# Woody5962/Ranked-List-Truncation

Hardware: AMD Instinct MI355X
Metric: ranked-lists/sec (fwd+bwd) at len=300; F1@k vs CPU ref (higher is better)
Workload: dtype f32 (operands, accumulation, storage); products by exact 3xbf16 split, 6 MFMA products, per-product error < 2^-23; 1 GPU; AttnCut + DivLoss(js,f1,augmented) [BASELINE configs[1]], batch 4096 lists/GPU x len 300, full train step incl. Adam and cut metrics; global_batch=4096, seq_len=300, parallelism=dp1

## Files before the change

include/rlt_hip.h:

```cpp
#ifndef RLT_HIP_H
#define RLT_HIP_H

#include <stddef.h>
#include <stdint.h>

#ifdef __cplusplus
extern "C" {
#endif

#define RLT_E_ARG      (-1)
#define RLT_E_SHAPE    (-2)
#define RLT_E_WORKSPACE (-3)
#define RLT_E_ALIGN    (-4)

#define RLT_ABI_VERSION 5
int rlt_abi_version(void);
#define RLT_PRECISION_DEFAULT (-1)
#define RLT_PRECISION_FP32   0
#define RLT_PRECISION_BF16X3 1
#define RLT_PRECISION_BF16X6 2
int rlt_set_precision(int mode);
int rlt_get_precision(void);
const char* rlt_error_string(int code);

#define RLT_METRIC_F1  0
#define RLT_METRIC_DCG 1
#define RLT_LOSS_EXPECT 0
#define RLT_LOSS_CE     1
#define RLT_LOSS_KL     2
#define RLT_LOSS_JS     3
int rlt_reward_loss(const float* p, const float* labels, const float* dcg_coef, int B, int S,
                    int metric, int kind, float tau,
                    float* loss_per_list, float* loss_out, float* dp, void* stream);
int rlt_reward_loss_ex(const float* p, const float* labels, const float* dcg_coef, int B, int S,
                       int metric, float penalty, int kind, float tau,
                       float* loss_per_list, float* loss_out, float* dp, void* stream);
int rlt_reward_matrix(const float* labels, const float* dcg_coef, int B, int S, int metric, float tau,
                      float* r_out, float* q_out, void* stream);
int rlt_reward_matrix_ex(const float* labels, const float* dcg_coef, int B, int S, int metric, float penalty, float tau,
                         float* r_out, float* q_out, void* stream);
size_t rlt_dcg_table_bytes(void);
int rlt_dcg_table_init(void* table, size_t table_bytes, void* stream);
size_t rlt_loss_metrics_workspace(int B);
int rlt_loss_metrics(const float* p, const float* labels, const float* dcg_coef, int B, int S,
                     int metric, float penalty, int kind, float tau, double metric_penalty,
                     float* loss_per_list, float* loss_out, float* dp,
                     int32_t* k_out, double* f1_out, double* dcg_out, double* sums,
                     const void* dcg_table, void* ws, size_t ws_bytes, void* stream);

size_t rlt_mt_terms_workspace(int B, int S);
int rlt_mt_terms(const float* rerank, const float* cls, const float* labels, int B, int S, float margin,
                 float* terms, void* ws, size_t ws_bytes, void* stream);
int rlt_mt_terms_bwd(const float* cls, const float* labels, const float* terms, int B, int S,
                     float w_rerank, float w_class, const float* gscale,
                     float* d_rerank, float* d_class, void* stream);
int rlt_weighted_sum(const float* const* x, const float* w, int n, float* out, void* stream);

int rlt_cut_metrics(const float* p, const float* labels, const int32_t* k_in, int B, int S,
                    int32_t* k_out, double* f1_out, double* dcg_out, double* sums, void* stream);
int rlt_cut_metrics_ex(const float* p, const float* labels, const int32_t* k_in, int B, int S, double penalty,
                       int32_t* k_out, double* f1_out, double* dcg_out, double* sums, void* stream);

int rlt_task_metrics(const float* labels, const float* pred, int B, int S,
                     double* dcg_out, double* auc_out, double* sums, void* stream);

size_t rlt_truncation_curves_workspace(int B, int S);
int rlt_truncation_curves(const float* labels, int B, int S, double penalty, const void* dcg_table, int accumulate,
                          double* curves, double* best_f1, int32_t* best_f1_k, double* best_dcg, int32_t* best_dcg_k,
                          double* sums, void* ws, size_t ws_bytes, void* stream);

#define RLT_CUT_ARGMAX 0
#define RLT_CUT_PAIR   1
size_t rlt_cut_report_workspace(int B, int S);
int rlt_cut_report(const float* p, int rule, const float* labels, const float* dcg_coef, int B, int S, int metric, float penalty,
                   double metric_penalty, double tau, double sharpen, const void* dcg_table, int accumulate,
                   int32_t* k, float* p_k, float* margin, double* f1, double* dcg, double* best_f1, int32_t* best_f1_k,
                   double* best_dcg, int32_t* best_dcg_k, int32_t* better, double* hist, double* pred_curve, double* reward_curve,
                   double* sums, void* ws, size_t ws_bytes, void* stream);

#define RLT_GEMM_RELU       1
#define RLT_GEMM_ACCUMULATE 2
size_t rlt_gemm_workspace(int ta, int tb, int M, int N, int K);
int rlt_gemm(int ta, int tb, int M, int N, int K,
             const float* A, int lda, const float* B, int ldb, float* C, int ldc,
             const float* bias, const float* bias2, int flags,
             void* ws, size_t ws_bytes, int precision, void* stream);
int rlt_gemm_ex(int ta, int tb, int M, int N, int K,
                const float* A, int lda, const float* B, int ldb, float* C, int ldc,
                const float* bias, const float* bias2, int flags,
                const float* relu_mask, int ldmask, float mask_scale, float* colsum_a,
                float drop_p, uint32_t seed,
                void* ws, size_t ws_bytes, int precision, void* stream);

#define RLT_GEMM_NONE   0
#define RLT_GEMM_F32    1
#define RLT_GEMM_3      2
#define RLT_GEMM_3B     3
#define RLT_GEMM_6      4
#define RLT_GEMM_6B     5
#define RLT_GEMM_6C     6
#define RLT_GEMM_6E     7
#define RLT_GEMM_6S     8
typedef struct rlt_gemm_dispatch {
    int family, ta, tb, fast, persistent, ns, kchunk, slab_xcd, epilogue, narrow;
} rlt_gemm_dispatch;
int rlt_gemm_last_dispatch(rlt_gemm_dispatch* out);

size_t rlt_gemm_bits_words(int M, int N);
int rlt_gemm_bits(int ta, int tb, int M, int N, int K,
                  const float* A, int lda, const float* B, int ldb, float* C, int ldc,
                  const float* bias, int flags, float drop_p, uint32_t seed,
                  uint32_t* relu_bits_out, const uint32_t* mask_bits_in, float mask_scale,
                  int precision, void* stream);
size_t rlt_colsum_workspace(int T, int N);
int rlt_colsum(const float* X, int ldx, int T, int N, float* out, int accumulate,
               void* ws, size_t ws_bytes, void* stream);
int rlt_segment_colsum(const float* X, int ldx, int G, int R, int N, float* out, int ldo,
                       int accumulate, void* stream);

size_t rlt_narrow_dw_workspace(int T, int M);
int rlt_narrow_dw(const float* A, int lda, const float* X, int ldx, int I, int T, int M,
                  float* dW, float* db, void* ws, size_t ws_bytes, void* stream);
int rlt_relu_bwd(float* dX, const float* Y, size_t n, void* stream);
int rlt_scale(float* x, const float* scale, size_t n, void* stream);

int rlt_add_layernorm_fwd(const float* x, const float* r, const float* gamma, const float* beta,
                          int T, int E, float eps, float drop_p, uint32_t seed,
                          float* y, float* stats, void* stream);
size_t rlt_add_layernorm_bwd_workspace(int T, int E);
int rlt_add_layernorm_bwd(const float* x, const float* r, const float* gamma, const float* stats,
                          const float* dy, int T, int E, float drop_p, uint32_t seed,
                          float* dz, float* dr, float* dgamma, float* dbeta,
                          int accumulate, void* ws, size_t ws_bytes, void* stream);
int rlt_dropout_mask(uint32_t seed, size_t rows, int cols, float p, float* out, void* stream);

size_t rlt_list_attention_fwd_workspace(int S, int B, int H, int HD, float drop_p, int precision);
int rlt_list_attention_images_retained(int S, int B, int H, int HD, int precision);
int rlt_list_attention_fwd(const float* qkv, int S, int B, int H, int HD, float drop_p, uint32_t seed,
                           float* out, float* lse, void* images, size_t images_bytes, int precision, void* stream);
size_t rlt_list_attention_bwd_workspace(int S, int B, int H, int HD, float drop_p, int precision);
int rlt_list_attention_bwd(const float* qkv, const float* out, const float* dout, const float* lse,
                           int S, int B, int H, int HD, float drop_p, uint32_t seed, const void* images, float* dqkv,
                           void* ws, size_t ws_bytes, int precision, void* stream);
int rlt_list_attention_bwd_prepare(const float* out, const float* dout, const float* lse, int S, int B, int H, int HD, float drop_p,
                                   const void* images, void* ws, size_t ws_bytes, int precision, void* stream);
int rlt_list_attention_bwd_dkv(const float* qkv, const float* dout, const float* lse, const void* images, void* ws, size_t ws_bytes,
                               int S, int B, int H, int HD, float drop_p, uint32_t seed, float* dqkv, int precision, void* stream);
int rlt_list_attention_bwd_dq(const float* qkv, const float* dout, const float* lse, const void* images, void* ws, size_t ws_bytes,
                              int S, int B, int H, int HD, float drop_p, uint32_t seed, float* dqkv, int precision, void* stream);
#define RLT_ATTN_NONE           0
#define RLT_ATTN_F32            1
#define RLT_ATTN_F32_SB         2
#define RLT_ATTN_F32_OCC1       3
#define RLT_ATTN_F32_HD16       4
#define RLT_ATTN_X3             5
#define RLT_ATTN_X6             6
#define RLT_ATTN_X6_IMG         7
#define RLT_ATTN_X6_PP          8
#define RLT_ATTN_X6_PP_IMG      9
#define RLT_ATTN_X6_DKV1        10
#define RLT_ATTN_X6_DQ1         11
#define RLT_ATTN_X6N_2W         12
#define RLT_ATTN_X6N_2W_SEEDED  13
#define RLT_ATTN_X6N_PIPE       14
#define RLT_ATTN_X6H_PIPE       15
#define RLT_ATTN_PREP_Q      1
#define RLT_ATTN_PREP_K      2
#define RLT_ATTN_PREP_V      4
#define RLT_ATTN_PREP_DO     8
#define RLT_ATTN_PREP_SEEDS  16
#define RLT_ATTN_PREP_DELTA  32
#define RLT_ATTN_IMAGES_NONE    0
#define RLT_ATTN_IMAGES_X3_QKV  1
#define RLT_ATTN_IMAGES_X6_QKV  2
#define RLT_ATTN_IMAGES_X6N_KV  3
#define RLT_ATTN_IMAGES_X6H_KV  4
#define RLT_ATTN_WS_DELTA       0
#define RLT_ATTN_WS_X3_DO       1
#define RLT_ATTN_WS_X6_DO       2
#define RLT_ATTN_WS_X6N_BLOCKS  3
typedef struct rlt_attention_plan {
    int fwd, fwd_fixup, dkv, dq;
    int fwd_prepare, bwd_prepare, dkv_prepare, dq_prepare;
    int images_kind, images_retained, ws_kind;
    size_t images_bytes, flags_offset, flags_bytes;
    size_t delta_bytes, ws_extra_bytes, ws_bytes, ws_prepare_bytes, ws_part_bytes;
} rlt_attention_plan;
int rlt_list_attention_plan(int S, int B, int H, int HD, float drop_p, int have_images, int precision, rlt_attention_plan* out);
int rlt_attention_dropout_mask(uint32_t seed, int S, int B, int H, float p, float* out, void* stream);
int rlt_attention_dropout_mask_range(uint32_t seed, int pair0, int npair, int B, float p, float* out, void* stream);

int rlt_bilstm_rec_fwd(float* gates, const float* w_hh_fwd, const float* w_hh_rev, int S, int B,
                       float* h_out, float* c_out, int precision, void* stream);

int rlt_bilstm_rec_fwd_x(const float* x, int I, const float* w_ih_fwd, const float* b_ih_fwd, const float* b_hh_fwd,
                         const float* w_ih_rev, const float* b_ih_rev, const float* b_hh_rev,
                         const float* w_hh_fwd, const float* w_hh_rev, int S, int B,
                         float* gates, float* h_out, float* c_out, int precision, void* stream);
int rlt_bilstm_rec_bwd(float* gates, const float* c, const float* w_hh_fwd, const float* w_hh_rev,
                       const float* d_hout, int S, int B, int precision, void* stream);
#define RLT_LSTM_F32          1
#define RLT_LSTM_X3           2
#define RLT_LSTM_X6           3
#define RLT_LSTM_X6W_SINGLE   4
#define RLT_LSTM_X6W_HALVES   5
struct rlt_bilstm_rec_plan { int fwd, bwd, fwd_lists, bwd_lists; };
int rlt_bilstm_rec_plan(int B, int xin, int precision, struct rlt_bilstm_rec_plan* out);

#define RLT_OP_ENCODER_STASH   1
#define RLT_OP_ENCODER_FWD_WS  2
#define RLT_OP_ENCODER_BWD_WS  3
#define RLT_OP_BILSTM_STASH    4
#define RLT_OP_BILSTM_WS       5
size_t rlt_workspace_bytes(int op, int S, int B, int E, int H, int FF, int train_dropout, int precision);

typedef struct rlt_encoder_weights {
    const float *in_proj_weight, *in_proj_bias, *out_proj_weight, *out_proj_bias, *norm1_weight, *norm1_bias,
                *linear1_weight, *linear1_bias, *linear2_weight, *linear2_bias, *norm2_weight, *norm2_bias;
} rlt_encoder_weights;
typedef struct rlt_encoder_grads {
    float *in_proj_weight, *in_proj_bias, *out_proj_weight, *out_proj_bias, *norm1_weight, *norm1_bias,
          *linear1_weight, *linear1_bias, *linear2_weight, *linear2_bias, *norm2_weight, *norm2_bias;
} rlt_encoder_grads;
int rlt_encoder_layer_fwd(const float* x, const rlt_encoder_weights* w, int S, int B, int E, int H, int FF, float eps,
                          float drop_p, const uint32_t* seeds, float* y, void* stash, size_t stash_bytes,
                          void* ws, size_t ws_bytes, int precision, void* stream);
int rlt_encoder_layer_bwd(const float* x, const rlt_encoder_weights* w, int S, int B, int E, int H, int FF, float eps,
                          float drop_p, const uint32_t* seeds, const float* dy, const void* stash, size_t stash_bytes,
                          float* dx, const rlt_encoder_grads* g, void* ws, size_t ws_bytes, int precision, void* stream);

typedef struct rlt_lstm_layer_weights { const float *w_ih[2], *w_hh[2], *b_ih[2], *b_hh[2]; } rlt_lstm_layer_weights;
typedef struct rlt_lstm_layer_grads { float *w_ih[2], *w_hh[2], *b_ih[2], *b_hh[2]; } rlt_lstm_layer_grads;
int rlt_bilstm_fwd(const float* x, int I, const rlt_lstm_layer_weights* w, int S, int B, float* h_out,
                   void* stash, size_t stash_bytes, void* ws, size_t ws_bytes, int precision, void* stream);
int rlt_bilstm_bwd(const float* x, int I, const rlt_lstm_layer_weights* w, const float* h_out, const float* dh_out, int S, int B,
                   void* stash, size_t stash_bytes, float* dx, const rlt_lstm_layer_grads* g,
                   void* ws, size_t ws_bytes, int precision, void* stream);

size_t rlt_bilstm_generic_bytes(int stash, int S, int B, int I, int hidden);
int rlt_bilstm_generic_fwd(const float* x, int I, int hidden, const rlt_lstm_layer_weights* w, int S, int B, float* h_out,
                           void* stash, size_t stash_bytes, void* ws, size_t ws_bytes, int precision, void* stream);
int rlt_bilstm_generic_bwd(const float* x, int I, int hidden, const rlt_lstm_layer_weights* w, const float* h_out,
                           const float* dh_out, int S, int B, void* stash, size_t stash_bytes, float* dx,
                           const rlt_lstm_layer_grads* g, void* ws, size_t ws_bytes, int precision, void* stream);

#define RLT_SPARSE_CHUNK 256
typedef struct rlt_sparse_batch {
    const float* dense; const int32_t* ids; const int32_t* perm;
    const int64_t* indptr; const int32_t* indices; const float* values;
    const int64_t* col_ptr; const int32_t* col_rows; const float* col_vals;
    const int32_t *chunk_col, *chunk_ptr, *multi_cols;
    int Dn, n_docs, V, n_chunks, n_multi;
} rlt_sparse_batch;
size_t rlt_sparse_inproj_workspace(int S, int B, int Dn, int n_docs, int V, int n_chunks);
int rlt_sparse_inproj_fwd(const rlt_sparse_batch* sb, int S, int B, const float* wt_fwd, const float* wt_rev,
                          const float* b_ih_fwd, const float* b_hh_fwd, const float* b_ih_rev, const float* b_hh_rev,
                          float* gates, void* stream);
int rlt_sparse_inproj_bwd(const rlt_sparse_batch* sb, int S, int B, const float* dgates, float* dwt_fwd, float* dwt_rev,
                          float* db_ih_fwd, float* db_hh_fwd, float* db_ih_rev, float* db_hh_rev,
// ... 115 lines not shown
```

ranked-list-truncation_amd/csrc/gemm.hip:

```cpp
#include "common.h"
#include "gemm6s.h"
#include "split6.h"
#include <stdlib.h>
#include <string.h>
#include <type_traits>

namespace {

constexpr int BM = 128, BN = 128, LDT = 132;

struct GemmArgs {
    const float* A; const float* B; float* C;
    const float* bias; const float* bias2;
    int M, N, K, lda, ldb, ldc;
    int vecA, vecB;
    int flags;
    int kchunk;
    float* slab;
    int tiles_m, tiles_n;
    const float* mask; int ldmask;
    float* colsum;
    float* cs_slab;
    float drop_p; uint32_t drop_thr, seed;
    float mask_scale;
    int slab_xcd;
    uint32_t* bits_out;
    const uint32_t* bits_in;
    int ldbits;
};

inline void note_dispatch(int family, bool ta, bool tb, bool fast, bool persistent, const GemmArgs& g, int ns) {
    rlt_gemm_dispatch_rec = rlt_gemm_dispatch{family, ta ? 1 : 0, tb ? 1 : 0, fast ? 1 : 0, persistent ? 1 : 0,
                                              ns, g.kchunk, g.slab_xcd, 0, 0};
}

__device__ __forceinline__ void decode_block(const GemmArgs& g, int& bid, int& z) {
    const int nwg = g.tiles_m * g.tiles_n;
    const int id = blockIdx.x;
    if (g.slab_xcd) {
        const int xcd = id & 7, j = id >> 3, grp = j / nwg;
        z = grp * 8 + xcd;
        bid = j - grp * nwg;
    } else {
        const int q = nwg >> 3, r = nwg & 7, xcd = id & 7, j = id >> 3;
        bid = (xcd < r ? xcd * (q + 1) : r * (q + 1) + (xcd - r) * q) + j;
        z = blockIdx.z;
    }
}

__device__ __forceinline__ float gemm_epilogue(const GemmArgs& g, float v, float bv, int row, int col, const float* dst) {
    v += bv;
    if (g.flags & RLT_GEMM_ACCUMULATE) v += *dst;
    if (g.flags & RLT_GEMM_RELU) v = fmaxf(v, 0.f);
    if (g.mask) v = (g.mask[(size_t)row * g.ldmask + col] > 0.f) ? v * g.mask_scale : 0.f;
    if (g.drop_p > 0.f) v = rlt_keep(g.seed, (uint32_t)row, (uint32_t)col, g.drop_thr) ? v * (1.f / (1.f - g.drop_p)) : 0.f;
    return v;
}

template <bool KC, int BK, bool FAST>
__device__ __forceinline__ void load_tile(const float* __restrict__ P, int ld, int mn0, int k0, int MN, int Kend,
                                          bool vec, int tid, float4 (&reg)[BK / 8]) {
#pragma unroll
    for (int i = 0; i < BK / 8; ++i) {
        const int idx = tid + 256 * i;
        float4 v = make_float4(0.f, 0.f, 0.f, 0.f);
        if (FAST) {
            int r, c;
            bool ok;
            if (KC) { r = mn0 + idx / (BK / 4); c = k0 + 4 * (idx % (BK / 4)); ok = r < MN && c < Kend; r = min(r, MN - 1); c = min(c, Kend - 4); }
            else { r = k0 + (idx >> 5); c = mn0 + 4 * (idx & 31); ok = r < Kend && c < MN; r = min(r, Kend - 1); c = min(c, MN - 4); }
            (void)ok;
            v = *reinterpret_cast<const float4*>(P + (size_t)r * ld + c);
        } else if (KC) {
            const int row = mn0 + idx / (BK / 4), kk = k0 + 4 * (idx % (BK / 4));
            if (row < MN) {
                const float* src = P + (size_t)row * ld + kk;
                if (vec && kk + 3 < Kend) {
                    v = *reinterpret_cast<const float4*>(src);
                } else {
                    if (kk + 0 < Kend) v.x = src[0];
                    if (kk + 1 < Kend) v.y = src[1];
                    if (kk + 2 < Kend) v.z = src[2];
                    if (kk + 3 < Kend) v.w = src[3];
                }
            }
        } else {
            const int kk = k0 + (idx >> 5), col = mn0 + 4 * (idx & 31);
            if (kk < Kend) {
                const float* src = P + (size_t)kk * ld + col;
                if (vec && col + 3 < MN) {
                    v = *reinterpret_cast<const float4*>(src);
                } else {
                    if (col + 0 < MN) v.x = src[0];
                    if (col + 1 < MN) v.y = src[1];
                    if (col + 2 < MN) v.z = src[2];
                    if (col + 3 < MN) v.w = src[3];
                }
            }
        }
        reg[i] = v;
    }
}

template <bool KC, int BK>
__device__ __forceinline__ void mask_tile(float4 (&reg)[BK / 8], int tid, int mn0, int k0, int MN, int Kend) {
#pragma unroll
    for (int i = 0; i < BK / 8; ++i) {
        const int idx = tid + 256 * i;
        const bool ok = KC ? (mn0 + idx / (BK / 4) < MN && k0 + 4 * (idx % (BK / 4)) < Kend)
                           : (k0 + (idx >> 5) < Kend && mn0 + 4 * (idx & 31) < MN);
        reg[i] = make_float4(ok ? reg[i].x : 0.f, ok ? reg[i].y : 0.f, ok ? reg[i].z : 0.f, ok ? reg[i].w : 0.f);
    }
}

template <bool KC, int BK>
__device__ __forceinline__ void store_tile(float* __restrict__ T, int tid, const float4 (&reg)[BK / 8]) {
#pragma unroll
    for (int i = 0; i < BK / 8; ++i) {
        const int idx = tid + 256 * i;
        if (KC) {
            const int mn = idx / (BK / 4), k = 4 * (idx % (BK / 4));
            T[(k + 0) * LDT + mn] = reg[i].x;
            T[(k + 1) * LDT + mn] = reg[i].y;
            T[(k + 2) * LDT + mn] = reg[i].z;
            T[(k + 3) * LDT + mn] = reg[i].w;
        } else {
            const int k = idx >> 5, mn = 4 * (idx & 31);
            *reinterpret_cast<float4*>(&T[k * LDT + mn]) = reg[i];
        }
    }
}

template <bool V> struct BoolTag { static constexpr bool value = V; };
template <int NJ>
__device__ __forceinline__ void write_output_t(const GemmArgs& g, const f32x16 (&acc)[2][NJ], int rbase, int cbase,
                                               bool interior, int l31, int hh, int z) {
    const bool to_slab = g.slab != nullptr;
    float* out = to_slab ? g.slab + (size_t)z * g.M * g.N : g.C;
    const int ldo = to_slab ? g.N : g.ldc;
    const int rb = __builtin_amdgcn_readfirstlane(rbase), cb = __builtin_amdgcn_readfirstlane(cbase);
    const int loff = 4 * hh * ldo + l31;
    if (interior && g.drop_p <= 0.f) {
        auto tile = [&](auto f) {
#pragma unroll
            for (int j = 0; j < NJ; ++j) {
                const int col = cb + j * 32 + l31;
                float bv = 0.f;
                if (!to_slab) {
                    if (g.bias) bv += g.bias[col];
                    if (g.bias2) bv += g.bias2[col];
                }
#pragma unroll
                for (int i = 0; i < 2; ++i) {
#pragma unroll
                    for (int r = 0; r < 16; ++r) {
                        const int dr = (r & 3) + 8 * (r >> 2);
                        float* base = out + (size_t)(rb + i * 32 + dr) * ldo + (cb + j * 32);
                        base[loff] = f(acc[i][j][r] + bv, rb + i * 32 + dr + 4 * hh, col, base + loff);
                    }
                }
            }
        };
        const bool relu = g.flags & RLT_GEMM_RELU, accum = g.flags & RLT_GEMM_ACCUMULATE;
        if (to_slab || (!relu && !accum && !g.mask && !g.bits_in)) { tile([](float v, int, int, const float*) { return v; }); return; }
        if (relu && !accum && !g.mask && !g.bits_out && !g.bits_in) { tile([](float v, int, int, const float*) { return fmaxf(v, 0.f); }); return; }
        if (accum && !relu && !g.mask && !g.bits_in) { tile([](float v, int, int, const float* d) { return v + *d; }); return; }
        if (((g.bits_out && relu) || (g.bits_in && !relu)) && !accum && !g.mask && !to_slab) {
            const float sc = g.mask_scale;
            auto body = [&](auto wr_tag) {
            constexpr bool wr = decltype(wr_tag)::value;
#pragma unroll
            for (int j = 0; j < NJ; ++j) {
                const int col = cb + j * 32 + l31;
                float bv = 0.f;
                if (g.bias) bv += g.bias[col];
                if (g.bias2) bv += g.bias2[col];
#pragma unroll
                for (int i = 0; i < 2; ++i) {
                    const size_t widx = (size_t)((rb + i * 32) >> 5) * g.ldbits + (cb + j * 32);
                    uint32_t w = wr ? 0u : (g.bits_in + widx)[l31];
                    if (!wr) w >>= 4 * hh;
// ... 1113 lines not shown
                    else stash6c_part<BKC>(t1 + 3 * HB6, t2 + 3 * HB6, tid, sb, piece - 4);
                }
                __builtin_amdgcn_sched_barrier(0);
            }
        }
        if (STASH) fetch(fetch_ti);
    };

    fetch(0);
    if (want_cs) add_cs();
#pragma unroll
    for (int part = 0; part < 4; ++part) {
        stash6c_part<AKC>(lds, lds + KB6, tid, sa, part);
        stash6c_part<BKC>(lds + 3 * HB6, lds + KB6 + 3 * HB6, tid, sb, part);
    }
    if (PERSIST) decode_next();
    fetch(1);
    __syncthreads();

    int u = 0;
    int nslot = 0; (void)nslot;
    while (true) {
        for (int ti = 0; ti < nt; ++ti) {
            const int b0 = u, b1 = u == 2 ? 0 : u + 1, b2 = b1 == 2 ? 0 : b1 + 1;
            RLT_G6C_STAMP(nslot, 0);
            slot(BoolTag<false>{}, b0, 0, 0, false, 0);
            RLT_G6C_STAMP(nslot, 1);
            __syncthreads();
            RLT_G6C_STAMP(nslot, 2);
            ++nslot;
            RLT_G6C_STAMP(nslot, 0);
            slot(BoolTag<true>{}, b1, b2, b0, ti + 1 < nt || has_next, ti + 2);
            RLT_G6C_STAMP(nslot, 1);
            __syncthreads();
            RLT_G6C_STAMP(nslot, 2);
            ++nslot;
            u = b2;
        }
#ifdef RLT_G6C_NOSTORE
        if (acc[0][0][0] == 123.456f)
#endif
        write_output_t<4>(g, acc, m0 + wm * 64, n0 + wn * 128, true, l31, hh, zslab);
        if (!PERSIST || !has_next) break;
        m0 = nm0; n0 = nn0;
        decode_next();
#pragma unroll
        for (int i = 0; i < 2; ++i)
#pragma unroll
            for (int j = 0; j < 4; ++j)
#pragma unroll
                for (int r = 0; r < 16; ++r) acc[i][j][r] = 0.f;
    }
    if (want_cs) {
        float4* red = reinterpret_cast<float4*>(gsm);
        __syncthreads();
        red[tid] = csum;
        __syncthreads();
        if (tid < 64) {
            float4 t = red[4 * tid];
#pragma unroll
            for (int j = 1; j < 8; ++j) {
                const float4 o = red[(j >> 2) * 256 + 4 * tid + (j & 3)];
                t.x += o.x; t.y += o.y; t.z += o.z; t.w += o.w;
            }
            float* dst = (g.cs_slab ? g.cs_slab + (size_t)zslab * g.M : g.colsum) + m0 + 4 * tid;
            dst[0] = t.x; dst[1] = t.y; dst[2] = t.z; dst[3] = t.w;
        }
    }
}
template <bool TA, bool TB>
int launch_gemm6c(GemmArgs g, int ns, hipStream_t st) {
    const size_t shm = (size_t)3 * KB6 * sizeof(uint16_t);
    g.tiles_m = g.M / BM2; g.tiles_n = g.N / BN2;
    if constexpr (!TA) {
        static const int persist_wgs = [] { const char* e = getenv("RLT_GEMM6_PERSIST"); return e ? atoi(e) : 256; }();
        const long long tiles = (long long)g.tiles_m * g.tiles_n;
        if (persist_wgs > 0 && ns == 1 && tiles > persist_wgs && persist_wgs % 8 == 0) {
            int rc = rlt_allow_lds(gemm6c_kernel<TA, TB, true>, shm);
            if (rc) return rc;
            note_dispatch(RLT_GEMM_6C, TA, TB, true, true, g, ns);
            hipLaunchKernelGGL((gemm6c_kernel<TA, TB, true>), dim3(persist_wgs), dim3(512), shm, st, g);
            return RLT_LAUNCH_RESULT();
        }
    }
    int rc = rlt_allow_lds(gemm6c_kernel<TA, TB, false>, shm);
    if (rc) return rc;
    dim3 grid(g.tiles_m * g.tiles_n * (g.slab_xcd ? ns : 1), 1, g.slab_xcd ? 1 : ns);
    note_dispatch(RLT_GEMM_6C, TA, TB, true, false, g, ns);
    hipLaunchKernelGGL((gemm6c_kernel<TA, TB, false>), grid, dim3(512), shm, st, g);
    return RLT_LAUNCH_RESULT();
}

template <bool KC>
__device__ __forceinline__ size_t off6e(int tid, int ld) {
    if (KC) return (size_t)phys6(tid >> 2) * ld + 4 * (tid & 3);
    return (size_t)(4 * (tid & 3)) * ld + 4 * (tid >> 2);
}
template <bool KC>
__device__ __forceinline__ void load6e(const float* __restrict__ P, int ld, int i, float4& v) {
    v = *reinterpret_cast<const float4*>(P + (size_t)(KC ? 64 * i : i) * ld);
}
template <bool KC>
__device__ __forceinline__ int dst6e(int tid, int p) {
    const int x = tid & 3;
    const int pr = KC ? (tid >> 2) + 64 * p : ((((tid >> 2) * 4) & ~15) | (p << 2) | ((tid >> 2) & 3));
    return pr * 16 + 8 * ((x >> 1) ^ ((pr >> 3) & 1)) + 4 * (x & 1);
}
template <bool KC>
__device__ __forceinline__ void vals6e(const float4 (&v)[4], int p, float& a, float& b, float& c, float& d) {
    if (KC) { a = v[p].x; b = v[p].y; c = v[p].z; d = v[p].w; }
    else {
        const float* f0 = reinterpret_cast<const float*>(&v[0]);
        const float* f1 = reinterpret_cast<const float*>(&v[1]);
        const float* f2 = reinterpret_cast<const float*>(&v[2]);
        const float* f3 = reinterpret_cast<const float*>(&v[3]);
        a = f0[p]; b = f1[p]; c = f2[p]; d = f3[p];
    }
}

template <int NJ>
__device__ __forceinline__ void write_output_simple(const GemmArgs& g, const f32x16 (&acc)[2][NJ], int rbase, int cbase, int l31, int hh, int z) {
    const bool to_slab = g.slab != nullptr;
    float* out = to_slab ? g.slab + (size_t)z * g.M * g.N : g.C;
    const int ldo = to_slab ? g.N : g.ldc;
    const int rb = __builtin_amdgcn_readfirstlane(rbase), cb = __builtin_amdgcn_readfirstlane(cbase);
    const int loff = 4 * hh * ldo + l31;
    const bool relu = !to_slab && (g.flags & RLT_GEMM_RELU), accum = !to_slab && (g.flags & RLT_GEMM_ACCUMULATE);
#pragma unroll
    for (int j = 0; j < NJ; ++j) {
        const int col = cb + j * 32 + l31;
        float bv = 0.f;
        if (!to_slab) {
            if (g.bias) bv += g.bias[col];
            if (g.bias2) bv += g.bias2[col];
        }
#pragma unroll
        for (int i = 0; i < 2; ++i) {
#pragma unroll
            for (int r = 0; r < 16; ++r) {
                const int dr = (r & 3) + 8 * (r >> 2);
                float* base = out + (size_t)(rb + i * 32 + dr) * ldo + (cb + j * 32);
                float v = acc[i][j][r] + bv;
                if (accum) v += base[loff];
                if (relu) v = fmaxf(v, 0.f);
                base[loff] = v;
            }
        }
    }
}
inline bool gemm6e_epilogue_ok(const GemmArgs& g) {
    return !g.mask && !g.bits_in && !g.bits_out && g.drop_p <= 0.f;
}

template <bool TA, bool TB, bool PERSIST>
__global__ __launch_bounds__(256, 1) void gemm6e_kernel(GemmArgs g) {
    extern __shared__ __attribute__((aligned(16))) float gsm[];
    uint16_t* lds = reinterpret_cast<uint16_t*>(gsm);
    const int tid = threadIdx.x, lane = tid & 63, wv = __builtin_amdgcn_readfirstlane(tid >> 6);
    const int l31 = lane & 31, hh = lane >> 5;
    const int wm = wv >> 1, wn = wv & 1;
    int bid, zslab;
    decode_block(g, bid, zslab);
    const int tm = bid / g.tiles_n, tn = bid - tm * g.tiles_n;
    int m0 = tm * BM2, n0 = tn * BN2;
    const int kbeg = zslab * g.kchunk;
    const int kend = min(g.K, kbeg + g.kchunk);
    const int nks = (kend - kbeg) / 16;

    f32x16 acc[2][2][4];
#pragma unroll
    for (int i = 0; i < 4; ++i)
#pragma unroll
        for (int j = 0; j < 4; ++j)
#pragma unroll
            for (int r = 0; r < 16; ++r) acc[i >> 1][i & 1][j][r] = 0.f;

    constexpr bool AKC = !TA, BKC = TB;
    const bool want_cs = TA && g.colsum != nullptr && tn == 0;
    float4 csum = make_float4(0.f, 0.f, 0.f, 0.f);
    const int pl = phys6(l31);
    const int csw = 8 * (hh ^ ((pl >> 3) & 1));
    const int arow = (wm * 128 + pl) * 16 + csw, brow = 3 * HB6 + (wn * 128 + pl) * 16 + csw;
    const size_t offA = off6e<AKC>(tid, g.lda), offB = off6e<BKC>(tid, g.ldb);
    int dA[4], dB[4];
#pragma unroll
    for (int p = 0; p < 4; ++p) { dA[p] = dst6e<AKC>(tid, p); dB[p] = 3 * HB6 + dst6e<BKC>(tid, p); }

    int vid = blockIdx.x, nm0 = m0, nn0 = n0;
    bool has_next = false;
    auto decode_next = [&]() {
        const int nwg = g.tiles_m * g.tiles_n;
        vid += gridDim.x;
        has_next = PERSIST && vid < nwg;
        if (has_next) {
            const int q = nwg >> 3, r = nwg & 7, xcd = vid & 7, jj = vid >> 3;
            const int nb = (xcd < r ? xcd * (q + 1) : r * (q + 1) + (xcd - r) * q) + jj;
            const int ntm = nb / g.tiles_n;
            nm0 = ntm * BM2; nn0 = (nb - ntm * g.tiles_n) * BN2;
        }
    };
    auto srcA = [&](int ks) {
        const bool wrap = PERSIST && has_next && ks >= nks;
        const int k0 = kbeg + 16 * (wrap ? ks - nks : min(ks, nks - 1)), mm = wrap ? nm0 : m0;
        return g.A + (AKC ? (size_t)mm * g.lda + k0 : (size_t)k0 * g.lda + mm) + offA;
    };
    auto srcB = [&](int ks) {
        const bool wrap = PERSIST && has_next && ks >= nks;
        const int k0 = kbeg + 16 * (wrap ? ks - nks : min(ks, nks - 1)), nn = wrap ? nn0 : n0;
        return g.B + (BKC ? (size_t)nn * g.ldb + k0 : (size_t)k0 * g.ldb + nn) + offB;
    };
    float4 ra[2][4], rb[2][4];
    auto add_cs = [&](const float4 (&v)[4]) {
#pragma unroll
        for (int i = 0; i < 4; ++i) { csum.x += v[i].x; csum.y += v[i].y; csum.z += v[i].z; csum.w += v[i].w; }
    };
    auto stash_all = [&](uint16_t* wb, const float4 (&va)[4], const float4 (&vb)[4]) {
#pragma unroll
        for (int p = 0; p < 4; ++p) {
            float a, b, c, d;
            uint2 hi, mid, lo;
            vals6e<AKC>(va, p, a, b, c, d);
            split4x3(a, b, c, d, hi, mid, lo);
            *reinterpret_cast<uint2*>(wb + dA[p]) = hi;
            *reinterpret_cast<uint2*>(wb + dA[p] + HB6) = mid;
            *reinterpret_cast<uint2*>(wb + dA[p] + 2 * HB6) = lo;
            vals6e<BKC>(vb, p, a, b, c, d);
            split4x3(a, b, c, d, hi, mid, lo);
            *reinterpret_cast<uint2*>(wb + dB[p]) = hi;
            *reinterpret_cast<uint2*>(wb + dB[p] + HB6) = mid;
            *reinterpret_cast<uint2*>(wb + dB[p] + 2 * HB6) = lo;
        }
    };
    bf16x8 a[4][3], b[2][3];
    auto frag_a = [&](const uint16_t* base, int i, int q) { a[i][q] = *reinterpret_cast<const bf16x8*>(base + arow + q * HB6 + i * 32 * 16); };
    auto frag_b = [&](const uint16_t* base, int j, int q) { b[j & 1][q] = *reinterpret_cast<const bf16x8*>(base + brow + q * HB6 + j * 32 * 16); };

    {
        const float* pa = srcA(0); const float* pb = srcB(0);
#pragma unroll
        for (int i = 0; i < 4; ++i) { load6e<AKC>(pa, g.lda, i, ra[0][i]); load6e<BKC>(pb, g.ldb, i, rb[0][i]); }
        pa = srcA(1); pb = srcB(1);
#pragma unroll
        for (int i = 0; i < 4; ++i) { load6e<AKC>(pa, g.lda, i, ra[1][i]); load6e<BKC>(pb, g.ldb, i, rb[1][i]); }
        if (want_cs) { add_cs(ra[0]); add_cs(ra[1]); }
        stash_all(lds, ra[0], rb[0]);
        stash_all(lds + KB6, ra[1], rb[1]);
        if (PERSIST) decode_next();
        pa = srcA(2); pb = srcB(2);
#pragma unroll
        for (int i = 0; i < 4; ++i) { load6e<AKC>(pa, g.lda, i, ra[0][i]); load6e<BKC>(pb, g.ldb, i, rb[0][i]); }
        pa = srcA(3); pb = srcB(3);
#pragma unroll
        for (int i = 0; i < 4; ++i) { load6e<AKC>(pa, g.lda, i, ra[1][i]); load6e<BKC>(pb, g.ldb, i, rb[1][i]); }
    }
    __syncthreads();
#pragma unroll
    for (int q = 0; q < 3; ++q) { frag_a(lds, 0, q); frag_a(lds, 1, q); frag_b(lds, 0, q); }

    auto slot = [&](auto par_tag, int buf, int wbuf, int nbuf, const float* pa, const float* pb) {
        constexpr int PAR = decltype(par_tag)::value;
        const uint16_t* base = lds + buf * KB6;
        const uint16_t* nbase = lds + nbuf * KB6;
        uint16_t* wb = lds + wbuf * KB6;
        Split6 su;
#define GAP_END __builtin_amdgcn_sched_barrier(0)
#define MM(i_, j_, k_) acc[(i_) >> 1][(i_) & 1][j_] = __builtin_amdgcn_mfma_f32_32x32x16_bf16( \
            a[i_][(k_) == 0 || (k_) == 3 ? 1 : (k_) == 1 ? 2 : 0], b[(j_) & 1][(k_) == 0 || (k_) == 4 ? 1 : (k_) == 2 ? 2 : 0], acc[(i_) >> 1][(i_) & 1][j_], 0, 0, 0)
#define SP(p_, k_) do { float x0_, x1_, x2_, x3_; \
            if ((p_) < 4) vals6e<AKC>(ra[PAR], (p_) & 3, x0_, x1_, x2_, x3_); else vals6e<BKC>(rb[PAR], (p_) & 3, x0_, x1_, x2_, x3_); \
            split6_part(su, x0_, x1_, x2_, x3_, k_); } while (0)
#define ST(p_) do { const int d_ = (p_) < 4 ? dA[(p_) & 3] : dB[(p_) & 3]; \
            *reinterpret_cast<uint2*>(wb + d_) = su.hi; *reinterpret_cast<uint2*>(wb + d_ + HB6) = su.mid; \
            *reinterpret_cast<uint2*>(wb + d_ + 2 * HB6) = su.lo; \
            if ((p_) < 4) { if (AKC) load6e<AKC>(pa, g.lda, (p_) & 3, ra[PAR][(p_) & 3]); \
                            else if ((p_) == 3) { for (int i_ = 0; i_ < 4; ++i_) load6e<AKC>(pa, g.lda, i_, ra[PAR][i_]); } } \
            else { if (BKC) load6e<BKC>(pb, g.ldb, (p_) & 3, rb[PAR][(p_) & 3]); \
                   else if ((p_) == 7) { for (int i_ = 0; i_ < 4; ++i_) load6e<BKC>(pb, g.ldb, i_, rb[PAR][i_]); } } } while (0)
#define RA(i_, q_, n_) frag_a((n_) ? nbase : base, i_, q_)
#define RB(j_, q_, n_) frag_b((n_) ? nbase : base, j_, q_)
#include "gemm6e_slot.inc"
#undef GAP_END
#undef MM
#undef SP
#undef ST
#undef RA
#undef RB
    };

    int u = 0;
    while (true) {
        for (int s = 0; s < nks; s += 2) {
            const int u1 = u == 2 ? 0 : u + 1, u2 = u1 == 2 ? 0 : u1 + 1;
            if (want_cs && s + 2 < nks) add_cs(ra[0]);
            slot(std::integral_constant<int, 0>{}, u, u2, u1, srcA(s + 4), srcB(s + 4));
            __syncthreads();
            if (want_cs && s + 3 < nks) add_cs(ra[1]);
            slot(std::integral_constant<int, 1>{}, u1, u, u2, srcA(s + 5), srcB(s + 5));
            __syncthreads();
            u = u2;
        }
        write_output_simple<4>(g, acc[0], m0 + wm * 128, n0 + wn * 128, l31, hh, zslab);
        write_output_simple<4>(g, acc[1], m0 + wm * 128 + 64, n0 + wn * 128, l31, hh, zslab);
        if (!PERSIST || !has_next) break;
        m0 = nm0; n0 = nn0;
        decode_next();
#pragma unroll
        for (int i = 0; i < 4; ++i)
#pragma unroll
            for (int j = 0; j < 4; ++j)
#pragma unroll
                for (int r = 0; r < 16; ++r) acc[i >> 1][i & 1][j][r] = 0.f;
    }
    if (want_cs) {
        float4* red = reinterpret_cast<float4*>(gsm);
        __syncthreads();
        red[tid] = csum;
        __syncthreads();
        if (tid < 64) {
            float4 t = red[4 * tid];
#pragma unroll
            for (int j = 1; j < 4; ++j) {
                const float4 o = red[4 * tid + j];
                t.x += o.x; t.y += o.y; t.z += o.z; t.w += o.w;
            }
            float* dst = (g.cs_slab ? g.cs_slab + (size_t)zslab * g.M : g.colsum) + m0 + 4 * tid;
            dst[0] = t.x; dst[1] = t.y; dst[2] = t.z; dst[3] = t.w;
        }
    }
}
template <bool TA, bool TB>
int launch_gemm6e(GemmArgs g, int ns, hipStream_t st) {
    const size_t shm = (size_t)3 * KB6 * sizeof(uint16_t);
    g.tiles_m = g.M / BM2; g.tiles_n = g.N / BN2;
    if constexpr (!TA) {
        static const int persist_wgs = [] { const char* e = getenv("RLT_GEMM6_PERSIST"); return e ? atoi(e) : 256; }();
        const long long tiles = (long long)g.tiles_m * g.tiles_n;
        if (persist_wgs > 0 && ns == 1 && tiles > persist_wgs && persist_wgs % 8 == 0) {
            int rc = rlt_allow_lds(gemm6e_kernel<TA, TB, true>, shm);
            if (rc) return rc;
            note_dispatch(RLT_GEMM_6E, TA, TB, true, true, g, ns);
            hipLaunchKernelGGL((gemm6e_kernel<TA, TB, true>), dim3(persist_wgs), dim3(256), shm, st, g);
            return RLT_LAUNCH_RESULT();
        }
    }
    int rc = rlt_allow_lds(gemm6e_kernel<TA, TB, false>, shm);
    if (rc) return rc;
    dim3 grid(g.tiles_m * g.tiles_n * (g.slab_xcd ? ns : 1), 1, g.slab_xcd ? 1 : ns);
    note_dispatch(RLT_GEMM_6E, TA, TB, true, false, g, ns);
    hipLaunchKernelGGL((gemm6e_kernel<TA, TB, false>), grid, dim3(256), shm, st, g);
    return RLT_LAUNCH_RESULT();
}

bool gemm6_ok(const GemmArgs& g) {
    if (!g.vecA || !g.vecB) return false;
    return !((g.M % BM6) || (g.N % BN6) || (g.K % BK3) || (g.kchunk % BK3));
}
template <bool TA, bool TB>
int launch_gemm6(GemmArgs g, int ns, hipStream_t st) {
    const size_t shm = (size_t)2 * BUF6 * sizeof(uint16_t);
    g.tiles_m = g.M / BM6; g.tiles_n = g.N / BN6;
    int rc = rlt_allow_lds(gemm6_kernel<TA, TB>, shm);
    if (rc) return rc;
    dim3 grid(g.tiles_m * g.tiles_n * (g.slab_xcd ? ns : 1), 1, g.slab_xcd ? 1 : ns);
    note_dispatch(RLT_GEMM_6, TA, TB, true, false, g, ns);
    hipLaunchKernelGGL((gemm6_kernel<TA, TB>), grid, dim3(512), shm, st, g);
    return RLT_LAUNCH_RESULT();
}

template <bool TA, bool TB, bool FAST>
int launch_gemm3_v(const GemmArgs& g, dim3 grid, int ns, hipStream_t st) {
    const size_t shm = (size_t)2 * 4 * TILE3 * sizeof(uint16_t);
    int rc = rlt_allow_lds(gemm3_kernel<TA, TB, FAST>, shm);
    if (rc) return rc;
    note_dispatch(RLT_GEMM_3, TA, TB, FAST, false, g, ns);
    hipLaunchKernelGGL((gemm3_kernel<TA, TB, FAST>), grid, dim3(256), shm, st, g);
    return RLT_LAUNCH_RESULT();
}
bool gemm_fast_ok(const GemmArgs& g, bool ta, bool tb);
template <bool TA, bool TB>
int launch_gemm3(const GemmArgs& g, dim3 grid, int ns, hipStream_t st) {
    if (gemm_fast_ok(g, TA, TB)) return launch_gemm3_v<TA, TB, true>(g, grid, ns, st);
    return launch_gemm3_v<TA, TB, false>(g, grid, ns, st);
}

__device__ __forceinline__ float4 f4add(float4 a, float4 b) { return make_float4(a.x + b.x, a.y + b.y, a.z + b.z, a.w + b.w); }
__global__ __launch_bounds__(256) void splitk_reduce_kernel(GemmArgs g, int nsplit) {
    const size_t mn = (size_t)g.M * g.N;
    const size_t stride = (size_t)gridDim.x * 256;
    if ((g.N & 3) == 0) {
        const float4* slab4 = reinterpret_cast<const float4*>(g.slab);
        const size_t mn4 = mn / 4;
        for (size_t i = (size_t)blockIdx.x * 256 + threadIdx.x; i < mn4; i += stride) {
            float4 a0 = make_float4(0.f, 0.f, 0.f, 0.f), a1 = a0, a2 = a0, a3 = a0;
            int z = 0;
            for (; z + 3 < nsplit; z += 4) {
                a0 = f4add(a0, slab4[(size_t)z * mn4 + i]);
                a1 = f4add(a1, slab4[(size_t)(z + 1) * mn4 + i]);
                a2 = f4add(a2, slab4[(size_t)(z + 2) * mn4 + i]);
                a3 = f4add(a3, slab4[(size_t)(z + 3) * mn4 + i]);
            }
            for (; z < nsplit; ++z) a0 = f4add(a0, slab4[(size_t)z * mn4 + i]);
            const float4 v4 = f4add(f4add(a0, a1), f4add(a2, a3));
            const float v[4] = {v4.x, v4.y, v4.z, v4.w};
            const int row = (int)((4 * i) / g.N), col0 = (int)(4 * i - (size_t)row * g.N);
#pragma unroll
            for (int e = 0; e < 4; ++e) {
                const int col = col0 + e;
                float bv = 0.f;
                if (g.bias) bv += g.bias[col];
                if (g.bias2) bv += g.bias2[col];
                float* dst = g.C + (size_t)row * g.ldc + col;
                *dst = gemm_epilogue(g, v[e], bv, row, col, dst);
            }
        }
    } else {
        for (size_t i = (size_t)blockIdx.x * 256 + threadIdx.x; i < mn; i += stride) {
            float v = 0.f;
            for (int z = 0; z < nsplit; ++z) v += g.slab[(size_t)z * mn + i];
            const int row = (int)(i / g.N), col = (int)(i - (size_t)row * g.N);
            float bv = 0.f;
            if (g.bias) bv += g.bias[col];
            if (g.bias2) bv += g.bias2[col];
            float* dst = g.C + (size_t)row * g.ldc + col;
            *dst = gemm_epilogue(g, v, bv, row, col, dst);
        }
    }
    if (g.cs_slab)
        for (size_t i = (size_t)blockIdx.x * 256 + threadIdx.x; i < (size_t)g.M; i += stride) {
            float c0 = 0.f, c1 = 0.f, c2 = 0.f, c3 = 0.f;
            int z = 0;
            for (; z + 3 < nsplit; z += 4) {
                c0 += g.cs_slab[(size_t)z * g.M + i];
                c1 += g.cs_slab[(size_t)(z + 1) * g.M + i];
                c2 += g.cs_slab[(size_t)(z + 2) * g.M + i];
                c3 += g.cs_slab[(size_t)(z + 3) * g.M + i];
            }
            for (; z < nsplit; ++z) c0 += g.cs_slab[(size_t)z * g.M + i];
            g.colsum[i] = (c0 + c1) + (c2 + c3);
        }
}

template <bool TA, bool TB, int BK, int OCC, bool FAST>
int launch_gemm_v(const GemmArgs& g, dim3 grid, int ns, hipStream_t st) {
    const size_t shm = (size_t)4 * BK * LDT * sizeof(float);
    int rc = rlt_allow_lds(gemm_kernel<TA, TB, BK, OCC, FAST>, shm);
    if (rc) return rc;
    note_dispatch(RLT_GEMM_F32, TA, TB, FAST, false, g, ns);
    hipLaunchKernelGGL((gemm_kernel<TA, TB, BK, OCC, FAST>), grid, dim3(256), shm, st, g);
    return RLT_LAUNCH_RESULT();
}
bool gemm_fast_ok(const GemmArgs& g, bool ta, bool tb) {
    static const int off = [] { const char* e = getenv("RLT_GEMM_NOFAST"); return e ? atoi(e) : 0; }();
    if (off) return false;
    if (!g.vecA || !g.vecB || (g.K & 3) || g.K < 4) return false;
    if (ta && ((g.M & 3) || g.M < 4)) return false;
    if (!tb && ((g.N & 3) || g.N < 4)) return false;
    return true;
}
template <bool TA, bool TB, int BK>
int launch_gemm(const GemmArgs& g, dim3 grid, int ns, hipStream_t st) {
    if (gemm_fast_ok(g, TA, TB)) return launch_gemm_v<TA, TB, BK, 4, true>(g, grid, ns, st);
    return launch_gemm_v<TA, TB, BK, 4, false>(g, grid, ns, st);
}

int gemm_mode() {
    static const int forced = [] {
        const char* e = getenv("RLT_GEMM_MODE");
        if (!e) return -1;
        if (!strcmp(e, "bf16x6") || !strcmp(e, "2")) return 2;
        return (!strcmp(e, "bf16x3") || !strcmp(e, "1")) ? 1 : 0;
    }();
    return forced >= 0 ? forced : rlt_precision();
}

int choose_split(int M, int N, int K) {
    const long long tiles = (long long)rlt_cdiv(M, BM) * rlt_cdiv(N, BN);
    static const int kmin = [] { const char* e = getenv("RLT_GEMM_SPLIT_KMIN"); return e ? atoi(e) : 1024; }();
    if (tiles >= 256 || K < kmin) return 1;
    static const int target = [] { const char* e = getenv("RLT_GEMM_SPLIT_TARGET"); return e ? atoi(e) : 1024; }();
    long long want = target / tiles > 0 ? target / tiles : 1;
    const long long per = K >= 4096 ? 512 : 256;
    const long long maxs = K / per > 0 ? K / per : 1;
    if (want > maxs) want = maxs;
    if (want > 256) want = 256;
    if (want >= 8) want = want / 8 * 8;
    return (int)(want < 1 ? 1 : want);
}

#if defined(RLT_STAMPS)
extern "C" int rlt_debug_g6c_stamps(unsigned long long* host, size_t n) {
    return (int)hipMemcpyFromSymbol(host, HIP_SYMBOL(rlt_g6c_stamp_buf), n * sizeof(unsigned long long));
}
extern "C" int rlt_debug_gemm_stamps(unsigned long long* host, size_t n) {
    return (int)hipMemcpyFromSymbol(host, HIP_SYMBOL(rlt_gemm_stamp_buf), n * sizeof(unsigned long long));
}
#endif

constexpr int CS_ROWS_PER_WG = 512;
__global__ __launch_bounds__(256) void colsum_partial_kernel(const float* __restrict__ X, int ldx, int T, int N,
                                                             float* __restrict__ partial) {
    const int col = blockIdx.x * 64 + (threadIdx.x & 63);
    const int rphase = threadIdx.x >> 6;
    const int r0 = blockIdx.y * CS_ROWS_PER_WG, r1 = min(T, r0 + CS_ROWS_PER_WG);
    float acc = 0.f;
    if (col < N)
        for (int r = r0 + rphase; r < r1; r += 4) acc += X[(size_t)r * ldx + col];
    __shared__ float sm[4][64];
    sm[rphase][threadIdx.x & 63] = acc;
    __syncthreads();
    if (threadIdx.x < 64 && col < N)
        partial[(size_t)blockIdx.y * N + col] = sm[0][threadIdx.x] + sm[1][threadIdx.x] + sm[2][threadIdx.x] + sm[3][threadIdx.x];
}
__global__ __launch_bounds__(256) void segment_colsum_kernel(const float* __restrict__ X, int ldx, int R, int N,
                                                             float* __restrict__ out, int ldo, int accumulate) {
    const int g = blockIdx.x;
    const int lane = threadIdx.x & 63, rphase = threadIdx.x >> 6;
    __shared__ float sm[4][64];
    for (int c0 = 0; c0 < N; c0 += 64) {
        const int col = c0 + lane;
        float acc = 0.f;
        if (col < N)
            for (int r = rphase; r < R; r += 4) acc += X[((size_t)g * R + r) * ldx + col];
        sm[rphase][lane] = acc;
        __syncthreads();
        if (threadIdx.x < 64 && col < N) {
            const float v = sm[0][lane] + sm[1][lane] + sm[2][lane] + sm[3][lane];
            float* dst = out + (size_t)g * ldo + col;
            *dst = accumulate ? *dst + v : v;
        }
        __syncthreads();
    }
}

__global__ __launch_bounds__(256) void relu_bwd_kernel(float* __restrict__ dX, const float* __restrict__ Y, size_t n) {
    for (size_t i = (size_t)blockIdx.x * 256 + threadIdx.x; i < n; i += (size_t)gridDim.x * 256)
        if (!(Y[i] > 0.f)) dX[i] = 0.f;
}
__global__ __launch_bounds__(256) void scale_kernel(float* __restrict__ x, const float* __restrict__ s, size_t n) {
    const float f = s[0];
    for (size_t i = (size_t)blockIdx.x * 256 + threadIdx.x; i < n; i += (size_t)gridDim.x * 256) x[i] *= f;
}

constexpr int NDW_CHUNKS = 2048;
__global__ __launch_bounds__(256) void narrow_dw_partial_kernel(const float* __restrict__ A, int lda, const float* __restrict__ X,
                                                                int ldx, int I, int T, int M, int rows_per_wg,
                                                                float* __restrict__ partial) {
    const int m4 = blockIdx.y * 256 + threadIdx.x;
    const int t0 = blockIdx.x * rows_per_wg, t1 = min(T, t0 + rows_per_wg);
    float4 a0 = make_float4(0.f, 0.f, 0.f, 0.f), a1 = a0, a2 = a0, ab = a0;
    if (4 * m4 < M) {
        const float* ap = A + 4 * m4;
        for (int t = t0; t < t1; ++t) {
            const float4 v = *reinterpret_cast<const float4*>(ap + (size_t)t * lda);
            const float* xr = X + (size_t)t * ldx;
            const float x0 = xr[0], x1 = I > 1 ? xr[1] : 0.f, x2 = I > 2 ? xr[2] : 0.f;
            a0.x += v.x * x0; a0.y += v.y * x0; a0.z += v.z * x0; a0.w += v.w * x0;
            a1.x += v.x * x1; a1.y += v.y * x1; a1.z += v.z * x1; a1.w += v.w * x1;
            a2.x += v.x * x2; a2.y += v.y * x2; a2.z += v.z * x2; a2.w += v.w * x2;
            ab.x += v.x; ab.y += v.y; ab.z += v.z; ab.w += v.w;
        }
        float* pr = partial + (size_t)blockIdx.x * 4 * M + 4 * m4;
        *reinterpret_cast<float4*>(pr) = a0;
        *reinterpret_cast<float4*>(pr + M) = a1;
        *reinterpret_cast<float4*>(pr + 2 * M) = a2;
        *reinterpret_cast<float4*>(pr + 3 * M) = ab;
    }
}
__global__ __launch_bounds__(256) void narrow_dw_scatter_kernel(const float* __restrict__ sums, int M, int I,
                                                                float* __restrict__ dW, float* __restrict__ db) {
    const int m = blockIdx.x * 256 + threadIdx.x;
    if (m >= M) return;
    for (int f = 0; f < I; ++f) dW[(size_t)m * I + f] = sums[(size_t)f * M + m];
    if (db) db[m] = sums[(size_t)3 * M + m];
}

int ew_grid(size_t n) { size_t g = (n + 1023) / 1024; return (int)(g < 1 ? 1 : (g > 4096 ? 4096 : g)); }

}

thread_local rlt_gemm_dispatch rlt_gemm_dispatch_rec = {};

extern "C" {

int rlt_gemm_last_dispatch(rlt_gemm_dispatch* out) {
    RLT_CHECK_ARG(out);
    *out = rlt_gemm_dispatch_rec;
    return 0;
}

size_t rlt_gemm_workspace(int ta, int tb, int M, int N, int K) {
    (void)ta; (void)tb;
    if (M <= 0 || N <= 0 || K <= 0) return 0;
    const int ns = choose_split(M, N, K);
    return ns > 1 ? ((size_t)ns * M * N + (size_t)ns * M) * sizeof(float) : 0;
}

int rlt_gemm(int ta, int tb, int M, int N, int K,
             const float* A, int lda, const float* B, int ldb, float* C, int ldc,
             const float* bias, const float* bias2, int flags,
             void* ws, size_t ws_bytes, int precision, void* stream) {
    RLT_PREC_SCOPE(precision);
    return rlt_gemm_ex(ta, tb, M, N, K, A, lda, B, ldb, C, ldc, bias, bias2, flags, nullptr, 0, 1.0f, nullptr,
                       0.0f, 0u, ws, ws_bytes, RLT_PRECISION_DEFAULT, stream);
}

static int gemm_run(int ta, int tb, int M, int N, int K,
                    const float* A, int lda, const float* B, int ldb, float* C, int ldc,
                    const float* bias, const float* bias2, int flags,
                    const float* relu_mask, int ldmask, float mask_scale, float* colsum_a,
                    float drop_p, uint32_t seed, uint32_t* bits_out, const uint32_t* bits_in,
                    void* ws, size_t ws_bytes, void* stream) {
    rlt_gemm_dispatch_rec = rlt_gemm_dispatch{};
    RLT_CHECK_ARG(A && B && C && M > 0 && N > 0 && K > 0);
    RLT_CHECK_ARG(lda >= (ta ? M : K) && ldb >= (tb ? K : N) && ldc >= N);
    RLT_CHECK_ARG(!relu_mask || ldmask >= N);
    RLT_CHECK_ARG(!colsum_a || ta);
    GemmArgs g;
    RLT_CHECK_ARG(drop_p >= 0.f && drop_p < 1.f);
    g.mask = relu_mask; g.ldmask = ldmask; g.colsum = colsum_a; g.cs_slab = nullptr;
    g.bits_out = bits_out; g.bits_in = bits_in; g.ldbits = N;
    g.mask_scale = mask_scale; g.drop_p = drop_p; g.drop_thr = rlt_drop_threshold(drop_p); g.seed = seed;
    g.A = A; g.B = B; g.C = C; g.bias = bias; g.bias2 = bias2;
    g.M = M; g.N = N; g.K = K; g.lda = lda; g.ldb = ldb; g.ldc = ldc;
    g.vecA = (lda % 4 == 0) && rlt_aligned16(A);
    g.vecB = (ldb % 4 == 0) && rlt_aligned16(B);
    g.flags = flags;
    g.tiles_m = rlt_cdiv(M, BM); g.tiles_n = rlt_cdiv(N, BN);
    int ns = (bits_out || bits_in) ? 1 : choose_split(M, N, K);
    if (ns > 1 && (!ws || ws_bytes < ((size_t)ns * M * N + (size_t)ns * M) * sizeof(float))) {
        if (ws == nullptr && ws_bytes == 0) ns = 1; else return RLT_E_WORKSPACE;
    }
    int kchunk = rlt_cdiv(rlt_cdiv(K, ns), 32) * 32;
    ns = rlt_cdiv(K, kchunk);
    g.kchunk = kchunk;
    static const bool no_slab_xcd = getenv("RLT_GEMM_NO_SLAB_XCD") != nullptr;
    g.slab_xcd = (ns > 1 && ns % 8 == 0 && !no_slab_xcd) ? 1 : 0;
    g.slab = ns > 1 ? (float*)ws : nullptr;
    g.cs_slab = (ns > 1 && colsum_a) ? (float*)ws + (size_t)ns * M * N : nullptr;
    hipStream_t st = rlt_stream(stream);
    dim3 grid(g.tiles_m * g.tiles_n * (g.slab_xcd ? ns : 1), 1, g.slab_xcd ? 1 : ns);
    int rc = 0;
    if (gemm_mode() == 2 && !ta && ns == 1 && !relu_mask && !colsum_a && drop_p == 0.f && !(flags & RLT_GEMM_ACCUMULATE) &&
        (!bits_in || (!bias && !bias2 && !(flags & RLT_GEMM_RELU)))) {
        const Gemm6sArgs s6{A, B, C, bias, bias2, M, N, K, lda, ldb, ldc, bits_out, bits_in, mask_scale};
        if (rlt_gemm6s_ok(s6)) {
            rc = rlt_gemm6s_launch(s6, tb != 0, (flags & RLT_GEMM_RELU) != 0, stream);
            return rc ? rc : RLT_LAUNCH_RESULT();
        }
    }
    static const bool x6_small_only = getenv("RLT_GEMM6_SMALL") != nullptr;
    static const bool x6_no_c = [] { const char* e = getenv("RLT_GEMM6C"); return e && atoi(e) == 0; }();
    if (gemm_mode() == 2 && gemm6_ok(g) && g.N % BN2 == 0 && !x6_small_only && !x6_no_c && g.kchunk / BK3 >= 2 &&
        (min(g.K, g.kchunk) / BK3) >= 2 && (g.K % g.kchunk == 0 || (g.K % g.kchunk) / BK3 >= 2)) {
        static const bool x6_e = [] { const char* e = getenv("RLT_GEMM6E"); return !e || atoi(e) != 0; }();
        static const bool x6_e_all = [] { const char* e = getenv("RLT_GEMM6E_ALL"); return e && atoi(e) != 0; }();
        if (x6_e && gemm6e_epilogue_ok(g) && (ta || g.K >= 1024 || x6_e_all)) {
            if (!ta && tb) rc = launch_gemm6e<false, true>(g, ns, st);
            else if (!ta && !tb) rc = launch_gemm6e<false, false>(g, ns, st);
            else if (!tb) rc = launch_gemm6e<true, false>(g, ns, st);
            else rc = launch_gemm6e<true, true>(g, ns, st);
        } else if (!ta && tb) rc = launch_gemm6c<false, true>(g, ns, st);
        else if (!ta && !tb) rc = launch_gemm6c<false, false>(g, ns, st);
        else if (ta && !tb) rc = launch_gemm6c<true, false>(g, ns, st);
        else rc = launch_gemm6c<true, true>(g, ns, st);
    } else if (gemm_mode() == 2 && gemm6_ok(g) && g.N % BN2 == 0 && !x6_small_only) {
        if (!ta && tb) rc = launch_gemm6b<false, true>(g, ns, st);
        else if (!ta && !tb) rc = launch_gemm6b<false, false>(g, ns, st);
        else if (ta && !tb) rc = launch_gemm6b<true, false>(g, ns, st);
        else rc = launch_gemm6b<true, true>(g, ns, st);
    } else if (gemm_mode() == 2 && gemm6_ok(g)) {
        if (!ta && tb) rc = launch_gemm6<false, true>(g, ns, st);
        else if (!ta && !tb) rc = launch_gemm6<false, false>(g, ns, st);
        else if (ta && !tb) rc = launch_gemm6<true, false>(g, ns, st);
        else rc = launch_gemm6<true, true>(g, ns, st);
    } else if (gemm_mode() == 1 && gemm_big_ok(g, ta, tb)) {
        if (!ta && tb) rc = launch_gemm3b<false, true>(g, ns, st);
        else if (!ta && !tb) rc = launch_gemm3b<false, false>(g, ns, st);
        else if (ta && !tb) rc = launch_gemm3b<true, false>(g, ns, st);
        else rc = launch_gemm3b<true, true>(g, ns, st);
    } else if (gemm_mode() == 1) {
        if (!ta && tb) rc = launch_gemm3<false, true>(g, grid, ns, st);
        else if (!ta && !tb) rc = launch_gemm3<false, false>(g, grid, ns, st);
        else if (ta && !tb) rc = launch_gemm3<true, false>(g, grid, ns, st);
        else rc = launch_gemm3<true, true>(g, grid, ns, st);
    } else {
        if (!ta && tb) rc = launch_gemm<false, true, 16>(g, grid, ns, st);
        else if (!ta && !tb) rc = launch_gemm<false, false, 16>(g, grid, ns, st);
        else if (ta && !tb) rc = launch_gemm<true, false, 16>(g, grid, ns, st);
        else rc = launch_gemm<true, true, 16>(g, grid, ns, st);
    }
    if (rc) return rc;
    if (ns > 1)
        hipLaunchKernelGGL(splitk_reduce_kernel, dim3(ew_grid((size_t)M * N)), dim3(256), 0, st, g, ns);
    return RLT_LAUNCH_RESULT();
}

int rlt_gemm_ex(int ta, int tb, int M, int N, int K,
                const float* A, int lda, const float* B, int ldb, float* C, int ldc,
                const float* bias, const float* bias2, int flags,
                const float* relu_mask, int ldmask, float mask_scale, float* colsum_a,
                float drop_p, uint32_t seed,
                void* ws, size_t ws_bytes, int precision, void* stream) {
    RLT_PREC_SCOPE(precision);
    return gemm_run(ta, tb, M, N, K, A, lda, B, ldb, C, ldc, bias, bias2, flags, relu_mask, ldmask, mask_scale, colsum_a,
                    drop_p, seed, nullptr, nullptr, ws, ws_bytes, stream);
}

size_t rlt_gemm_bits_words(int M, int N) { return M > 0 && N > 0 ? (size_t)rlt_cdiv(M, 32) * N : 0; }

int rlt_gemm_bits(int ta, int tb, int M, int N, int K,
                  const float* A, int lda, const float* B, int ldb, float* C, int ldc,
                  const float* bias, int flags, float drop_p, uint32_t seed,
                  uint32_t* relu_bits_out, const uint32_t* mask_bits_in, float mask_scale,
                  int precision, void* stream) {
    RLT_PREC_SCOPE(precision);
    RLT_CHECK_ARG((relu_bits_out != nullptr) != (mask_bits_in != nullptr));
    RLT_CHECK_ARG(!relu_bits_out || (flags & RLT_GEMM_RELU));
    RLT_CHECK_ARG(drop_p == 0.f || relu_bits_out);
    RLT_CHECK_SHAPE(N % 32 == 0);
    return gemm_run(ta, tb, M, N, K, A, lda, B, ldb, C, ldc, bias, nullptr, flags, nullptr, 0, mask_scale, nullptr,
                    drop_p, seed, relu_bits_out, mask_bits_in, nullptr, 0, stream);
}

size_t rlt_colsum_workspace(int T, int N) {
    if (T <= 0 || N <= 0) return 0;
    return (size_t)rlt_cdiv(T, CS_ROWS_PER_WG) * N * sizeof(float);
}

int rlt_colsum(const float* X, int ldx, int T, int N, float* out, int accumulate,
               void* ws, size_t ws_bytes, void* stream) {
    RLT_CHECK_ARG(X && out && ws && T > 0 && N > 0 && ldx >= N);
    if (ws_bytes < rlt_colsum_workspace(T, N)) return RLT_E_WORKSPACE;
    const int nchunk = rlt_cdiv(T, CS_ROWS_PER_WG);
    hipStream_t st = rlt_stream(stream);
    hipLaunchKernelGGL(colsum_partial_kernel, dim3(rlt_cdiv(N, 64), nchunk), dim3(256), 0, st, X, ldx, T, N, (float*)ws);
    hipLaunchKernelGGL(rlt_rows_reduce_kernel, dim3(rlt_cdiv(N, 16)), dim3(256), 0, st, (const float*)ws, nchunk, N, N, N, out, out, accumulate);
    return RLT_LAUNCH_RESULT();
}

int rlt_segment_colsum(const float* X, int ldx, int G, int R, int N, float* out, int ldo,
                       int accumulate, void* stream) {
    RLT_CHECK_ARG(X && out && G > 0 && R > 0 && N > 0 && ldx >= N && ldo >= N);
    hipLaunchKernelGGL(segment_colsum_kernel, dim3(G), dim3(256), 0, rlt_stream(stream), X, ldx, R, N, out, ldo, accumulate);
    return RLT_LAUNCH_RESULT();
}

size_t rlt_narrow_dw_workspace(int T, int M) {
    if (T <= 0 || M <= 0) return 0;
    const int rows = rlt_cdiv(T, NDW_CHUNKS);
    const int nchunk = rlt_cdiv(T, rows);
    return ((size_t)nchunk * 4 * M + (size_t)4 * M) * sizeof(float);
}

int rlt_narrow_dw(const float* A, int lda, const float* X, int ldx, int I, int T, int M,
                  float* dW, float* db, void* ws, size_t ws_bytes, void* stream) {
    RLT_CHECK_ARG(A && X && dW && ws && T > 0 && M > 0 && lda >= M && ldx >= I);
    RLT_CHECK_SHAPE(I >= 1 && I <= 3 && M % 4 == 0 && lda % 4 == 0);
    if (!rlt_aligned16(A)) return RLT_E_ALIGN;
    if (ws_bytes < rlt_narrow_dw_workspace(T, M)) return RLT_E_WORKSPACE;
    const int rows = rlt_cdiv(T, NDW_CHUNKS);
    const int nchunk = rlt_cdiv(T, rows);
    float* partial = (float*)ws;
    float* sums = partial + (size_t)nchunk * 4 * M;
    hipStream_t st = rlt_stream(stream);
    hipLaunchKernelGGL(narrow_dw_partial_kernel, dim3(nchunk, rlt_cdiv(M, 1024)), dim3(256), 0, st, A, lda, X, ldx, I, T, M, rows, partial);
    hipLaunchKernelGGL(rlt_rows_reduce_kernel, dim3(rlt_cdiv(4 * M, 16)), dim3(256), 0, st, (const float*)partial, nchunk, 4 * M,
                       4 * M, 4 * M, sums, sums, 0);
    hipLaunchKernelGGL(narrow_dw_scatter_kernel, dim3(rlt_cdiv(M, 256)), dim3(256), 0, st, (const float*)sums, M, I, dW, db);
    return RLT_LAUNCH_RESULT();
}

int rlt_relu_bwd(float* dX, const float* Y, size_t n, void* stream) {
    RLT_CHECK_ARG(dX && Y && n > 0);
    hipLaunchKernelGGL(relu_bwd_kernel, dim3(ew_grid(n)), dim3(256), 0, rlt_stream(stream), dX, Y, n);
    return RLT_LAUNCH_RESULT();
}

int rlt_scale(float* x, const float* scale, size_t n, void* stream) {
    RLT_CHECK_ARG(x && scale && n > 0);
    hipLaunchKernelGGL(scale_kernel, dim3(ew_grid(n)), dim3(256), 0, rlt_stream(stream), x, scale, n);
    return RLT_LAUNCH_RESULT();
}

}
```

ranked-list-truncation_amd/csrc/path.hip:

```cpp
#include "common.h"
#include <stdio.h>
#include <stdlib.h>

namespace {

constexpr size_t ALIGN = 256;
inline size_t rup(size_t b) { return (b + ALIGN - 1) / ALIGN * ALIGN; }

struct Cursor {
    uint8_t* base; size_t off, cap;
    explicit Cursor(void* p, size_t cap_ = (size_t)-1) : base((uint8_t*)p), off(0), cap(cap_) {}
    template <typename T = float> T* take(size_t bytes) {
        T* p = (T*)(base ? base + off : nullptr);
#ifdef RLT_BOUNDS_CHECK
        if (base && cap != (size_t)-1 && off + bytes > cap) {
            fprintf(stderr, "rlt bounds check: region of %zu bytes at offset %zu leaves a %zu-byte buffer\n", bytes, off, cap);
            abort();
        }
#endif
        off += rup(bytes);
        return p;
    }
};

struct EncDims { int S, B, E, H, FF; size_t T; int HD; bool bits; };

inline int enc_dims(int S, int B, int E, int H, int FF, EncDims& d) {
    if (S <= 0 || B <= 0 || E <= 0 || H <= 0 || FF <= 0 || E % H) return RLT_E_ARG;
    d = EncDims{S, B, E, H, FF, (size_t)S * B, E / H, FF % 32 == 0};
    if ((size_t)S * B > 0x7fffffffu) return RLT_E_SHAPE;
    return 0;
}

struct EncStash {
    float *qkv, *att, *lse, *proj, *st1, *h1, *hid, *ff, *st2;
    uint32_t* bits;
    void* images; size_t images_bytes;
    size_t bytes;
};
inline EncStash enc_stash(const EncDims& d, void* base, size_t cap = (size_t)-1) {
    Cursor c(base, cap);
    EncStash s{};
    const size_t T = d.T, f = sizeof(float);
    s.qkv = c.take(T * 3 * d.E * f);
    s.att = c.take(T * d.E * f);
    s.lse = c.take((size_t)d.S * d.H * d.B * f);
    s.proj = c.take(T * d.E * f);
    s.st1 = c.take(T * 2 * f);
    s.h1 = c.take(T * d.E * f);
    s.hid = c.take(T * d.FF * f);
    s.bits = d.bits ? c.take<uint32_t>(rlt_gemm_bits_words((int)T, d.FF) * sizeof(uint32_t)) : nullptr;
    s.ff = c.take(T * d.E * f);
    s.st2 = c.take(T * 2 * f);
    const bool keep = rlt_list_attention_images_retained(d.S, d.B, d.H, d.HD, RLT_PRECISION_DEFAULT) != 0;
    s.images_bytes = keep ? rlt_list_attention_fwd_workspace(d.S, d.B, d.H, d.HD, 0.f, RLT_PRECISION_DEFAULT) : 0;
    s.images = s.images_bytes ? c.take<uint8_t>(s.images_bytes) : nullptr;
    s.bytes = c.off;
    return s;
}
inline size_t enc_fwd_images_scratch(const EncDims& d, float drop_p) {
    if (rlt_list_attention_images_retained(d.S, d.B, d.H, d.HD, RLT_PRECISION_DEFAULT)) return 0;
    return rlt_list_attention_fwd_workspace(d.S, d.B, d.H, d.HD, drop_p, RLT_PRECISION_DEFAULT);
}

struct EncScratch {
    float *dz2, *dr2, *dhid, *dr1, *datt, *dqkv;
    void *attn_ws, *ln_ws, *gemm_ws;
    size_t attn_ws_bytes, ln_ws_bytes, gemm_ws_bytes, bytes;
};
inline size_t enc_gemm_ws(const EncDims& d) {
    const int T = (int)d.T;
    size_t m = 0;
    auto up = [&](size_t v) { if (v > m) m = v; };
    up(rlt_gemm_workspace(1, 0, d.E, d.FF, T));
    up(rlt_gemm_workspace(1, 0, d.FF, d.E, T));
    up(rlt_gemm_workspace(1, 0, d.E, d.E, T));
    up(rlt_gemm_workspace(1, 0, 3 * d.E, d.E, T));
    up(rlt_gemm_workspace(0, 1, T, 3 * d.E, d.E));
    up(rlt_gemm_workspace(0, 1, T, d.FF, d.E));
    up(rlt_gemm_workspace(0, 1, T, d.E, d.FF));
    up(rlt_gemm_workspace(0, 0, T, d.FF, d.E));
    up(rlt_gemm_workspace(0, 0, T, d.E, d.FF));
    up(rlt_gemm_workspace(0, 0, T, d.E, 3 * d.E));
    return m;
}
inline EncScratch enc_scratch(const EncDims& d, bool drop, void* base, size_t cap = (size_t)-1) {
    Cursor c(base, cap);
    EncScratch w{};
    const size_t T = d.T, f = sizeof(float);
    w.dz2 = c.take(T * d.E * f);
    w.dr2 = drop ? c.take(T * d.E * f) : nullptr;
    const size_t mid = c.off;
    w.dhid = c.take(T * d.FF * f);
    const size_t end_ffn = c.off;
    c.off = mid;
    w.dr1 = drop ? c.take(T * d.E * f) : nullptr;
    w.datt = c.take(T * d.E * f);
    w.dqkv = c.take(T * 3 * d.E * f);
    w.attn_ws_bytes = rlt_list_attention_bwd_workspace(d.S, d.B, d.H, d.HD, drop ? 0.5f : 0.f, RLT_PRECISION_DEFAULT);
    w.attn_ws = c.take<uint8_t>(w.attn_ws_bytes);
    if (c.off < end_ffn) c.off = end_ffn;
    w.ln_ws_bytes = rlt_add_layernorm_bwd_workspace((int)T, d.E);
    w.ln_ws = c.take<uint8_t>(w.ln_ws_bytes);
    w.gemm_ws_bytes = enc_gemm_ws(d);
    w.gemm_ws = c.take<uint8_t>(w.gemm_ws_bytes);
    w.bytes = c.off;
    return w;
}

#define RLT_TRY(expr) do { int rc_ = (expr); if (rc_) return rc_; } while (0)

inline int gemm(int ta, int tb, int M, int N, int K, const float* A, int lda, const float* B, int ldb, float* C, int ldc,
                const float* bias, int flags, float* colsum_a, void* ws, size_t ws_bytes, void* st) {
    return rlt_gemm_ex(ta, tb, M, N, K, A, lda, B, ldb, C, ldc, bias, nullptr, flags, nullptr, 0, 1.f, colsum_a, 0.f, 0u,
                       ws, ws_bytes, RLT_PRECISION_DEFAULT, st);
}

struct LstmStash { float *gates[2], *c[2], *h0; size_t bytes; };
inline LstmStash lstm_stash(size_t T, void* base, size_t cap = (size_t)-1) {
    Cursor cur(base, cap);
    LstmStash s{};
    for (int l = 0; l < 2; ++l) {
        s.gates[l] = cur.take(T * 1024 * sizeof(float));
        s.c[l] = cur.take(T * 256 * sizeof(float));
    }
    s.h0 = cur.take(T * 256 * sizeof(float));
    s.bytes = cur.off;
    return s;
}
struct LstmScratch { float *wcat, *bcat, *dh0, *dwcat, *dbcat; void* ws; size_t ws_bytes, bytes; };
inline LstmScratch lstm_scratch(size_t T, int I, void* base, size_t cap = (size_t)-1) {
    Cursor cur(base, cap);
    LstmScratch w{};
    const int Imax = I > 256 ? I : 256;
    w.wcat = cur.take((size_t)1024 * Imax * sizeof(float));
    w.bcat = cur.take(2 * 1024 * sizeof(float));
    w.dh0 = cur.take(T * 256 * sizeof(float));
    w.dwcat = cur.take((size_t)1024 * Imax * sizeof(float));
    w.dbcat = cur.take(1024 * sizeof(float));
    size_t m = rlt_narrow_dw_workspace((int)T, 1024);
    auto up = [&](size_t v) { if (v > m) m = v; };
    up(rlt_gemm_workspace(1, 0, 1024, Imax, (int)T));
    up(rlt_gemm_workspace(1, 0, 512, 128, (int)T));
    up(rlt_gemm_workspace(0, 1, (int)T, 1024, Imax));
    up(rlt_gemm_workspace(0, 0, (int)T, Imax, 1024));
    w.ws_bytes = m;
    w.ws = cur.take<uint8_t>(m);
    w.bytes = cur.off;
    return w;
}

__global__ __launch_bounds__(256) void pack2_kernel(const float* __restrict__ a, const float* __restrict__ b, size_t n,
                                                    float* __restrict__ out) {
    for (size_t i = (size_t)blockIdx.x * 256 + threadIdx.x; i < 2 * n; i += (size_t)gridDim.x * 256)
        out[i] = i < n ? a[i] : b[i - n];
}
__global__ __launch_bounds__(256) void unpack2_kernel(const float* __restrict__ in, size_t n, float* __restrict__ a,
                                                      float* __restrict__ b) {
    for (size_t i = (size_t)blockIdx.x * 256 + threadIdx.x; i < 2 * n; i += (size_t)gridDim.x * 256) {
        if (i < n) a[i] = in[i]; else b[i - n] = in[i];
    }
}
inline int pack2(const float* a, const float* b, size_t n, float* out, hipStream_t st) {
    const int grid = (int)((2 * n + 255) / 256 < 512 ? (2 * n + 255) / 256 : 512);
    hipLaunchKernelGGL(pack2_kernel, dim3(grid), dim3(256), 0, st, a, b, n, out);
    return RLT_LAUNCH_RESULT();
}
inline int unpack2(const float* in, size_t n, float* a, float* b, hipStream_t st) {
    const int grid = (int)((2 * n + 255) / 256 < 512 ? (2 * n + 255) / 256 : 512);
    hipLaunchKernelGGL(unpack2_kernel, dim3(grid), dim3(256), 0, st, in, n, a, b);
    return RLT_LAUNCH_RESULT();
}

int lstm_layer_fwd(const float* x, int I, const rlt_lstm_layer_weights& w, int S, int B, float* gates, float* c, float* h,
                   const LstmScratch& sc, void* stream, const rlt_sparse_batch* sp = nullptr) {
    const int T = S * B;
    if (sp) {
        RLT_TRY(rlt_sparse_inproj_fwd(sp, S, B, w.w_ih[0], w.w_ih[1], w.b_ih[0], w.b_hh[0], w.b_ih[1], w.b_hh[1], gates, stream));
        return rlt_bilstm_rec_fwd(gates, w.w_hh[0], w.w_hh[1], S, B, h, c, RLT_PRECISION_DEFAULT, stream);
    }
    if (I <= 3)
        return rlt_bilstm_rec_fwd_x(x, I, w.w_ih[0], w.b_ih[0], w.b_hh[0], w.w_ih[1], w.b_ih[1], w.b_hh[1], w.w_hh[0], w.w_hh[1],
                                    S, B, gates, h, c, RLT_PRECISION_DEFAULT, stream);
    hipStream_t st = rlt_stream(stream);
    RLT_TRY(pack2(w.w_ih[0], w.w_ih[1], (size_t)512 * I, sc.wcat, st));
    RLT_TRY(pack2(w.b_ih[0], w.b_ih[1], 512, sc.bcat, st));
    RLT_TRY(pack2(w.b_hh[0], w.b_hh[1], 512, sc.bcat + 1024, st));
    RLT_TRY(rlt_gemm_ex(0, 1, T, 1024, I, x, I, sc.wcat, I, gates, 1024, sc.bcat, sc.bcat + 1024, 0, nullptr, 0, 1.f, nullptr,
                        0.f, 0u, sc.ws, sc.ws_bytes, RLT_PRECISION_DEFAULT, stream));
    return rlt_bilstm_rec_fwd(gates, w.w_hh[0], w.w_hh[1], S, B, h, c, RLT_PRECISION_DEFAULT, stream);
}

int lstm_layer_bwd(const float* x, int I, const rlt_lstm_layer_weights& w, const float* h, float* gates, const float* c,
                   const float* dh, int S, int B, float* dx, const rlt_lstm_layer_grads& g, const LstmScratch& sc, void* stream,
                   const rlt_sparse_batch* sp = nullptr, void* sp_ws = nullptr, size_t sp_ws_bytes = 0) {
    const int T = S * B;
    hipStream_t st = rlt_stream(stream);
    RLT_TRY(rlt_bilstm_rec_bwd(gates, c, w.w_hh[0], w.w_hh[1], dh, S, B, RLT_PRECISION_DEFAULT, stream));
    const float* dA = gates;
    if (sp) {
        RLT_TRY(rlt_sparse_inproj_bwd(sp, S, B, dA, g.w_ih[0], g.w_ih[1], g.b_ih[0], g.b_hh[0], g.b_ih[1], g.b_hh[1],
                                      sp_ws, sp_ws_bytes, stream));
    } else if (I <= 3) {
        RLT_TRY(rlt_narrow_dw(dA, 1024, x, I, I, T, 1024, sc.dwcat, sc.dbcat, sc.ws, sc.ws_bytes, stream));
    } else {
        RLT_TRY(gemm(1, 0, 1024, I, T, dA, 1024, x, I, sc.dwcat, I, nullptr, 0, sc.dbcat, sc.ws, sc.ws_bytes, stream));
    }
    if (!sp) {
        RLT_TRY(unpack2(sc.dwcat, (size_t)512 * I, g.w_ih[0], g.w_ih[1], st));
        RLT_TRY(unpack2(sc.dbcat, 512, g.b_ih[0], g.b_ih[1], st));
        RLT_TRY(unpack2(sc.dbcat, 512, g.b_hh[0], g.b_hh[1], st));
    }
    if (S > 1) {
        const int K = T - B;
        RLT_TRY(gemm(1, 0, 512, 128, K, dA + (size_t)B * 1024, 1024, h, 256, g.w_hh[0], 128, nullptr, 0, nullptr, sc.ws, sc.ws_bytes, stream));
        RLT_TRY(gemm(1, 0, 512, 128, K, dA + 512, 1024, h + (size_t)B * 256 + 128, 256, g.w_hh[1], 128, nullptr, 0, nullptr, sc.ws, sc.ws_bytes, stream));
    } else {
        RLT_TRY((int)hipMemsetAsync(g.w_hh[0], 0, 512 * 128 * sizeof(float), st));
        RLT_TRY((int)hipMemsetAsync(g.w_hh[1], 0, 512 * 128 * sizeof(float), st));
    }
    if (dx) {
        RLT_TRY(pack2(w.w_ih[0], w.w_ih[1], (size_t)512 * I, sc.wcat, st));
        RLT_TRY(gemm(0, 0, T, I, 1024, dA, 1024, sc.wcat, I, dx, I, nullptr, 0, nullptr, sc.ws, sc.ws_bytes, stream));
    }
    return 0;
}

bool lstm_weights_ok(const rlt_lstm_layer_weights& w) {
    for (int d = 0; d < 2; ++d)
        if (!w.w_ih[d] || !w.w_hh[d] || !w.b_ih[d] || !w.b_hh[d]) return false;
    return true;
}
bool lstm_grads_ok(const rlt_lstm_layer_grads& g) {
    for (int d = 0; d < 2; ++d)
        if (!g.w_ih[d] || !g.w_hh[d] || !g.b_ih[d] || !g.b_hh[d]) return false;
    return true;
}

}

extern "C" {

size_t rlt_workspace_bytes(int op, int S, int B, int E, int H, int FF, int train_dropout, int precision) {
    RLT_PREC_SCOPE_SZ(precision);
    if (op == RLT_OP_ENCODER_STASH || op == RLT_OP_ENCODER_BWD_WS || op == RLT_OP_ENCODER_FWD_WS) {
        EncDims d;
        if (enc_dims(S, B, E, H, FF, d)) return 0;
        if (op == RLT_OP_ENCODER_STASH) return enc_stash(d, nullptr).bytes;
        if (op == RLT_OP_ENCODER_FWD_WS) return rup(enc_gemm_ws(d)) + rup(enc_fwd_images_scratch(d, train_dropout ? 0.5f : 0.f));
        return enc_scratch(d, train_dropout != 0, nullptr).bytes;
    }
    if (op == RLT_OP_BILSTM_STASH || op == RLT_OP_BILSTM_WS) {
        if (S <= 0 || B <= 0 || E <= 0) return 0;
        const size_t T = (size_t)S * B;
        return op == RLT_OP_BILSTM_STASH ? lstm_stash(T, nullptr).bytes : lstm_scratch(T, E, nullptr).bytes;
    }
    return 0;
}

int rlt_encoder_layer_fwd(const float* x, const rlt_encoder_weights* w, int S, int B, int E, int H, int FF, float eps,
                          float drop_p, const uint32_t* seeds, float* y, void* stash, size_t stash_bytes,
                          void* ws, size_t ws_bytes, int precision, void* stream) {
    RLT_PREC_SCOPE(precision);
    RLT_CHECK_ARG(x && w && y && stash && drop_p >= 0.f && drop_p < 1.f && (drop_p == 0.f || seeds));
    RLT_CHECK_ARG(w->in_proj_weight && w->in_proj_bias && w->out_proj_weight && w->out_proj_bias && w->norm1_weight &&
                  w->norm1_bias && w->linear1_weight && w->linear1_bias && w->linear2_weight && w->linear2_bias &&
                  w->norm2_weight && w->norm2_bias);
    EncDims d;
    RLT_TRY(enc_dims(S, B, E, H, FF, d));
    const size_t gemm_ws = rup(enc_gemm_ws(d)), img_scratch = enc_fwd_images_scratch(d, drop_p);
    if (stash_bytes < enc_stash(d, nullptr).bytes || ws_bytes < gemm_ws + img_scratch || (gemm_ws + img_scratch && !ws)) return RLT_E_WORKSPACE;
    EncStash s = enc_stash(d, stash, stash_bytes);
    if (img_scratch) { s.images = static_cast<uint8_t*>(ws) + gemm_ws; s.images_bytes = img_scratch; }
    const int T = (int)d.T;
    const uint32_t s_attn = drop_p > 0.f ? seeds[0] : 0u, s_ln1 = drop_p > 0.f ? seeds[1] : 0u,
                   s_ffn = drop_p > 0.f ? seeds[2] : 0u, s_ln2 = drop_p > 0.f ? seeds[3] : 0u;
    RLT_TRY(gemm(0, 1, T, 3 * E, E, x, E, w->in_proj_weight, E, s.qkv, 3 * E, w->in_proj_bias, 0, nullptr, ws, ws_bytes, stream));
    RLT_TRY(rlt_list_attention_fwd(s.qkv, S, B, H, d.HD, drop_p, s_attn, s.att, s.lse, s.images, s.images_bytes, RLT_PRECISION_DEFAULT, stream));
    RLT_TRY(gemm(0, 1, T, E, E, s.att, E, w->out_proj_weight, E, s.proj, E, w->out_proj_bias, 0, nullptr, ws, ws_bytes, stream));
    RLT_TRY(rlt_add_layernorm_fwd(x, s.proj, w->norm1_weight, w->norm1_bias, T, E, eps, drop_p, s_ln1, s.h1, s.st1, stream));
    if (d.bits) {
        RLT_TRY(rlt_gemm_bits(0, 1, T, FF, E, s.h1, E, w->linear1_weight, E, s.hid, FF, w->linear1_bias, RLT_GEMM_RELU,
                              drop_p, s_ffn, s.bits, nullptr, 1.f, RLT_PRECISION_DEFAULT, stream));
    } else {
        RLT_TRY(rlt_gemm_ex(0, 1, T, FF, E, s.h1, E, w->linear1_weight, E, s.hid, FF, w->linear1_bias, nullptr, RLT_GEMM_RELU,
                            nullptr, 0, 1.f, nullptr, drop_p, s_ffn, ws, ws_bytes, RLT_PRECISION_DEFAULT, stream));
    }
    RLT_TRY(gemm(0, 1, T, E, FF, s.hid, FF, w->linear2_weight, FF, s.ff, E, w->linear2_bias, 0, nullptr, ws, ws_bytes, stream));
    return rlt_add_layernorm_fwd(s.h1, s.ff, w->norm2_weight, w->norm2_bias, T, E, eps, drop_p, s_ln2, y, s.st2, stream);
}

int rlt_encoder_layer_bwd(const float* x, const rlt_encoder_weights* w, int S, int B, int E, int H, int FF, float eps,
                          float drop_p, const uint32_t* seeds, const float* dy, const void* stash, size_t stash_bytes,
                          float* dx, const rlt_encoder_grads* g, void* ws, size_t ws_bytes, int precision, void* stream) {
    RLT_PREC_SCOPE(precision);
    (void)eps;
    RLT_CHECK_ARG(x && w && dy && stash && dx && g && ws && drop_p >= 0.f && drop_p < 1.f && (drop_p == 0.f || seeds));
    RLT_CHECK_ARG(g->in_proj_weight && g->in_proj_bias && g->out_proj_weight && g->out_proj_bias && g->norm1_weight &&
                  g->norm1_bias && g->linear1_weight && g->linear1_bias && g->linear2_weight && g->linear2_bias &&
                  g->norm2_weight && g->norm2_bias);
    EncDims d;
    RLT_TRY(enc_dims(S, B, E, H, FF, d));
    const bool drop = drop_p > 0.f;
    if (stash_bytes < enc_stash(d, nullptr).bytes || ws_bytes < enc_scratch(d, drop, nullptr).bytes) return RLT_E_WORKSPACE;
    const EncStash s = enc_stash(d, const_cast<void*>(stash), stash_bytes);
    const EncScratch k = enc_scratch(d, drop, ws, ws_bytes);
    const int T = (int)d.T;
    const uint32_t s_attn = drop ? seeds[0] : 0u, s_ln1 = drop ? seeds[1] : 0u, s_ln2 = drop ? seeds[3] : 0u;
    const float keep_scale = 1.f / (1.f - drop_p);
    RLT_TRY(rlt_add_layernorm_bwd(s.h1, s.ff, w->norm2_weight, s.st2, dy, T, E, drop_p, s_ln2, k.dz2, k.dr2,
                                  g->norm2_weight, g->norm2_bias, 0, k.ln_ws, k.ln_ws_bytes, stream));
    const float* dr2 = drop ? k.dr2 : k.dz2;
    RLT_TRY(gemm(1, 0, E, FF, T, dr2, E, s.hid, FF, g->linear2_weight, FF, nullptr, 0, g->linear2_bias, k.gemm_ws, k.gemm_ws_bytes, stream));
    if (d.bits) {
        RLT_TRY(rlt_gemm_bits(0, 0, T, FF, E, dr2, E, w->linear2_weight, FF, k.dhid, FF, nullptr, 0, 0.f, 0u, nullptr, s.bits,
                              keep_scale, RLT_PRECISION_DEFAULT, stream));
    } else {
        RLT_TRY(rlt_gemm_ex(0, 0, T, FF, E, dr2, E, w->linear2_weight, FF, k.dhid, FF, nullptr, nullptr, 0, s.hid, FF, keep_scale,
                            nullptr, 0.f, 0u, k.gemm_ws, k.gemm_ws_bytes, RLT_PRECISION_DEFAULT, stream));
    }
    RLT_TRY(gemm(1, 0, FF, E, T, k.dhid, FF, s.h1, E, g->linear1_weight, E, nullptr, 0, g->linear1_bias, k.gemm_ws, k.gemm_ws_bytes, stream));
    RLT_TRY(gemm(0, 0, T, E, FF, k.dhid, FF, w->linear1_weight, E, k.dz2, E, nullptr, RLT_GEMM_ACCUMULATE, nullptr, k.gemm_ws, k.gemm_ws_bytes, stream));
    RLT_TRY(rlt_add_layernorm_bwd(x, s.proj, w->norm1_weight, s.st1, k.dz2, T, E, drop_p, s_ln1, dx, k.dr1,
                                  g->norm1_weight, g->norm1_bias, 0, k.ln_ws, k.ln_ws_bytes, stream));
    const float* dr1 = drop ? k.dr1 : dx;
    RLT_TRY(gemm(1, 0, E, E, T, dr1, E, s.att, E, g->out_proj_weight, E, nullptr, 0, g->out_proj_bias, k.gemm_ws, k.gemm_ws_bytes, stream));
    RLT_TRY(gemm(0, 0, T, E, E, dr1, E, w->out_proj_weight, E, k.datt, E, nullptr, 0, nullptr, k.gemm_ws, k.gemm_ws_bytes, stream));
    RLT_TRY(rlt_list_attention_bwd(s.qkv, s.att, k.datt, s.lse, S, B, H, d.HD, drop_p, s_attn, s.images, k.dqkv,
                                   k.attn_ws, k.attn_ws_bytes, RLT_PRECISION_DEFAULT, stream));
    RLT_TRY(gemm(1, 0, 3 * E, E, T, k.dqkv, 3 * E, x, E, g->in_proj_weight, E, nullptr, 0, g->in_proj_bias, k.gemm_ws, k.gemm_ws_bytes, stream));
    return gemm(0, 0, T, E, 3 * E, k.dqkv, 3 * E, w->in_proj_weight, E, dx, E, nullptr, RLT_GEMM_ACCUMULATE, nullptr, k.gemm_ws, k.gemm_ws_bytes, stream);
}

int rlt_bilstm_fwd(const float* x, int I, const rlt_lstm_layer_weights* w, int S, int B, float* h_out,
                   void* stash, size_t stash_bytes, void* ws, size_t ws_bytes, int precision, void* stream) {
    RLT_PREC_SCOPE(precision);
    RLT_CHECK_ARG(x && w && h_out && stash && ws && I > 0 && S > 0 && B > 0 && lstm_weights_ok(w[0]) && lstm_weights_ok(w[1]));
    const size_t T = (size_t)S * B;
    RLT_CHECK_SHAPE(T <= 0x7fffffffu);
    if (stash_bytes < lstm_stash(T, nullptr).bytes || ws_bytes < lstm_scratch(T, I, nullptr).bytes) return RLT_E_WORKSPACE;
    const LstmStash s = lstm_stash(T, stash, stash_bytes);
    const LstmScratch k = lstm_scratch(T, I, ws, ws_bytes);
    RLT_TRY(lstm_layer_fwd(x, I, w[0], S, B, s.gates[0], s.c[0], s.h0, k, stream));
    return lstm_layer_fwd(s.h0, 256, w[1], S, B, s.gates[1], s.c[1], h_out, k, stream);
}

int rlt_bilstm_bwd(const float* x, int I, const rlt_lstm_layer_weights* w, const float* h_out, const float* dh_out, int S, int B,
                   void* stash, size_t stash_bytes, float* dx, const rlt_lstm_layer_grads* g,
                   void* ws, size_t ws_bytes, int precision, void* stream) {
    RLT_PREC_SCOPE(precision);
    RLT_CHECK_ARG(x && w && h_out && dh_out && stash && g && ws && I > 0 && S > 0 && B > 0);
    RLT_CHECK_ARG(lstm_weights_ok(w[0]) && lstm_weights_ok(w[1]) && lstm_grads_ok(g[0]) && lstm_grads_ok(g[1]));
    const size_t T = (size_t)S * B;
    RLT_CHECK_SHAPE(T <= 0x7fffffffu);
    if (stash_bytes < lstm_stash(T, nullptr).bytes || ws_bytes < lstm_scratch(T, I, nullptr).bytes) return RLT_E_WORKSPACE;
    const LstmStash s = lstm_stash(T, stash, stash_bytes);
    const LstmScratch k = lstm_scratch(T, I, ws, ws_bytes);
    RLT_TRY(lstm_layer_bwd(s.h0, 256, w[1], h_out, s.gates[1], s.c[1], dh_out, S, B, k.dh0, g[1], k, stream));
    return lstm_layer_bwd(x, I, w[0], s.h0, s.gates[0], s.c[0], k.dh0, S, B, dx, g[0], k, stream);
}

size_t rlt_bilstm_sparse_workspace(int S, int B, int Dn, int n_docs, int V, int n_chunks) {
    const size_t sp = rlt_sparse_inproj_workspace(S, B, Dn, n_docs, V, n_chunks);
    if (!sp) return 0;
    return lstm_scratch((size_t)S * B, 256, nullptr).bytes + rup(sp);
}

int rlt_bilstm_sparse_fwd(const rlt_sparse_batch* sb, const rlt_lstm_layer_weights* w, int S, int B, float* h_out,
                          void* stash, size_t stash_bytes, void* ws, size_t ws_bytes, int precision, void* stream) {
    RLT_PREC_SCOPE(precision);
    RLT_CHECK_ARG(sb && w && h_out && stash && ws && S > 0 && B > 0 && lstm_weights_ok(w[0]) && lstm_weights_ok(w[1]));
    const size_t T = (size_t)S * B;
    RLT_CHECK_SHAPE(T <= 0x7fffffffu);
    if (stash_bytes < lstm_stash(T, nullptr).bytes || ws_bytes < lstm_scratch(T, 256, nullptr).bytes) return RLT_E_WORKSPACE;
    const LstmStash s = lstm_stash(T, stash, stash_bytes);
    const LstmScratch k = lstm_scratch(T, 256, ws, ws_bytes);
    RLT_TRY(lstm_layer_fwd(nullptr, 0, w[0], S, B, s.gates[0], s.c[0], s.h0, k, stream, sb));
    return lstm_layer_fwd(s.h0, 256, w[1], S, B, s.gates[1], s.c[1], h_out, k, stream);
}

int rlt_bilstm_sparse_bwd(const rlt_sparse_batch* sb, const rlt_lstm_layer_weights* w, const float* h_out, const float* dh_out,
                          int S, int B, void* stash, size_t stash_bytes, const rlt_lstm_layer_grads* g,
                          void* ws, size_t ws_bytes, int precision, void* stream) {
    RLT_PREC_SCOPE(precision);
    RLT_CHECK_ARG(sb && w && h_out && dh_out && stash && g && ws && S > 0 && B > 0);
    RLT_CHECK_ARG(lstm_weights_ok(w[0]) && lstm_weights_ok(w[1]) && lstm_grads_ok(g[0]) && lstm_grads_ok(g[1]));
    const size_t T = (size_t)S * B;
    RLT_CHECK_SHAPE(T <= 0x7fffffffu);
    const size_t sp_bytes = rlt_sparse_inproj_workspace(S, B, sb->Dn, sb->n_docs, sb->V, sb->n_chunks);
    RLT_CHECK_ARG(sp_bytes > 0);
    const size_t dense_bytes = lstm_scratch(T, 256, nullptr).bytes;
    if (stash_bytes < lstm_stash(T, nullptr).bytes || ws_bytes < dense_bytes + rup(sp_bytes)) return RLT_E_WORKSPACE;
    const LstmStash s = lstm_stash(T, stash, stash_bytes);
    const LstmScratch k = lstm_scratch(T, 256, ws, dense_bytes);
    RLT_TRY(lstm_layer_bwd(s.h0, 256, w[1], h_out, s.gates[1], s.c[1], dh_out, S, B, k.dh0, g[1], k, stream));
    return lstm_layer_bwd(nullptr, 0, w[0], s.h0, s.gates[0], s.c[0], k.dh0, S, B, nullptr, g[0], k, stream,
                          sb, static_cast<uint8_t*>(ws) + dense_bytes, sp_bytes);
}

}
```

ranked-list-truncation_amd/rlt_hip/native.py:

```python
import ctypes
import os
from ctypes import c_char_p, c_double, c_float, c_int, c_size_t, c_uint32, c_void_p

import torch

_PKG = os.path.dirname(os.path.dirname(os.path.abspath(__file__)))
LIB_PATH = os.environ.get("RLT_HIP_LIB") or os.path.join(_PKG, "csrc", "librlt_hip.so")

METRIC_F1, METRIC_DCG = 0, 1
LOSS_EXPECT, LOSS_CE, LOSS_KL, LOSS_JS = 0, 1, 2, 3
GEMM_RELU, GEMM_ACCUMULATE = 1, 2
HEAD_SOFTMAX, HEAD_SIGMOID, HEAD_IDENTITY = 0, 1, 2
PROBE_BCE, PROBE_RERANK = 0, 1
CUT_ARGMAX, CUT_PAIR = 0, 1
PRECISION_DEFAULT, PRECISION_FP32, PRECISION_BF16X3, PRECISION_BF16X6 = -1, 0, 1, 2
_PRECISION_NAMES = {PRECISION_FP32: "fp32", PRECISION_BF16X3: "bf16x3", PRECISION_BF16X6: "bf16x6"}

P = c_void_p
_SIGNATURES = {
    "rlt_abi_version": (c_int, []),
    "rlt_error_string": (c_char_p, [c_int]),
    "rlt_set_precision": (c_int, [c_int]),
    "rlt_get_precision": (c_int, []),
    "rlt_reward_loss": (c_int, [P, P, P, c_int, c_int, c_int, c_int, c_float, P, P, P, P]),
    "rlt_reward_matrix": (c_int, [P, P, c_int, c_int, c_int, c_float, P, P, P]),
    "rlt_reward_loss_ex": (c_int, [P, P, P, c_int, c_int, c_int, c_float, c_int, c_float, P, P, P, P]),
    "rlt_reward_matrix_ex": (c_int, [P, P, c_int, c_int, c_int, c_float, c_float, P, P, P]),
    "rlt_loss_metrics_workspace": (c_size_t, [c_int]),
    "rlt_dcg_table_bytes": (c_size_t, []),
    "rlt_dcg_table_init": (c_int, [P, c_size_t, P]),
    "rlt_loss_metrics": (c_int, [P, P, P, c_int, c_int, c_int, c_float, c_int, c_float, c_double, P, P, P, P, P, P, P, P, P, c_size_t, P]),
    "rlt_cut_metrics_ex": (c_int, [P, P, P, c_int, c_int, c_double, P, P, P, P, P]),
    "rlt_mt_terms_workspace": (c_size_t, [c_int, c_int]),
    "rlt_mt_terms": (c_int, [P, P, P, c_int, c_int, c_float, P, P, c_size_t, P]),
    "rlt_mt_terms_bwd": (c_int, [P, P, P, c_int, c_int, c_float, c_float, P, P, P, P]),
    "rlt_weighted_sum": (c_int, [P, P, c_int, P, P]),
    "rlt_cut_metrics": (c_int, [P, P, P, c_int, c_int, P, P, P, P, P]),
    "rlt_wass_loss_workspace": (c_size_t, [c_int, c_int]),
    "rlt_wass_loss_fwd": (c_int, [P, P, c_int, c_int, c_float, c_int, c_float, P, P, c_size_t, P]),
    "rlt_wass_loss_bwd": (c_int, [P, P, P, c_int, c_int, c_float, c_int, P, c_size_t, P, P]),
    "rlt_task_metrics": (c_int, [P, P, c_int, c_int, P, P, P, P]),
    "rlt_truncation_curves_workspace": (c_size_t, [c_int, c_int]),
    "rlt_truncation_curves": (c_int, [P, c_int, c_int, c_double, P, c_int, P, P, P, P, P, P, P, c_size_t, P]),
    "rlt_cut_report_workspace": (c_size_t, [c_int, c_int]),
    "rlt_cut_report": (c_int, [P, c_int, P, P, c_int, c_int, c_int, c_float, c_double, c_double, c_double, P, c_int,
                               P, P, P, P, P, P, P, P, P, P, P, P, P, P, P, c_size_t, P]),
    "rlt_probe_heads_workspace": (c_size_t, [c_int, c_int, c_int, c_int]),
    "rlt_probe_heads": (c_int, [P, P, P, P, c_int, c_int, c_int, c_int, P, c_float, P, P, P, P, P, c_size_t, P]),
    "rlt_neighbor_features": (c_int, [P, c_int, c_int, c_int, P, c_int, c_int, P, P, P, P, c_int, c_int, P]),
    "rlt_pair_softmax_fwd": (c_int, [P, c_int, c_int, c_float, c_uint32, P, P]),
    "rlt_pair_softmax_bwd": (c_int, [P, P, c_int, c_int, c_float, c_uint32, P, P]),
    "rlt_bicut_loss": (c_int, [P, P, c_int, c_int, c_int, c_float, c_float, P, P, P, P]),
    "rlt_gemm_workspace": (c_size_t, [c_int, c_int, c_int, c_int, c_int]),
    "rlt_gemm_bits_words": (c_size_t, [c_int, c_int]),
    "rlt_gemm_bits": (c_int, [c_int, c_int, c_int, c_int, c_int, P, c_int, P, c_int, P, c_int, P, c_int, c_float, c_uint32,
                              P, P, c_float, c_int, P]),
    "rlt_gemm": (c_int, [c_int, c_int, c_int, c_int, c_int, P, c_int, P, c_int, P, c_int, P, P, c_int, P, c_size_t, c_int, P]),
    "rlt_gemm_ex": (c_int, [c_int, c_int, c_int, c_int, c_int, P, c_int, P, c_int, P, c_int, P, P, c_int, P, c_int, c_float,
                            P, c_float, c_uint32, P, c_size_t, c_int, P]),
    "rlt_gemm_last_dispatch": (c_int, [P]),
    "rlt_dropout_mask": (c_int, [c_uint32, c_size_t, c_int, c_float, P, P]),
    "rlt_attention_dropout_mask": (c_int, [c_uint32, c_int, c_int, c_int, c_float, P, P]),
    "rlt_attention_dropout_mask_range": (c_int, [c_uint32, c_int, c_int, c_int, c_float, P, P]),
    "rlt_colsum_workspace": (c_size_t, [c_int, c_int]),
    "rlt_colsum": (c_int, [P, c_int, c_int, c_int, P, c_int, P, c_size_t, P]),
    "rlt_segment_colsum": (c_int, [P, c_int, c_int, c_int, c_int, P, c_int, c_int, P]),
    "rlt_narrow_dw_workspace": (c_size_t, [c_int, c_int]),
    "rlt_narrow_dw": (c_int, [P, c_int, P, c_int, c_int, c_int, c_int, P, P, P, c_size_t, P]),
    "rlt_relu_bwd": (c_int, [P, P, c_size_t, P]),
    "rlt_scale": (c_int, [P, P, c_size_t, P]),
    "rlt_add_layernorm_fwd": (c_int, [P, P, P, P, c_int, c_int, c_float, c_float, c_uint32, P, P, P]),
    "rlt_add_layernorm_bwd_workspace": (c_size_t, [c_int, c_int]),
    "rlt_add_layernorm_bwd": (c_int, [P, P, P, P, P, c_int, c_int, c_float, c_uint32, P, P, P, P, c_int, P, c_size_t, P]),
    "rlt_list_attention_fwd_workspace": (c_size_t, [c_int, c_int, c_int, c_int, c_float, c_int]),
    "rlt_list_attention_images_retained": (c_int, [c_int, c_int, c_int, c_int, c_int]),
    "rlt_list_attention_fwd": (c_int, [P, c_int, c_int, c_int, c_int, c_float, c_uint32, P, P, P, c_size_t, c_int, P]),
    "rlt_list_attention_bwd_workspace": (c_size_t, [c_int, c_int, c_int, c_int, c_float, c_int]),
    "rlt_list_attention_bwd": (c_int, [P, P, P, P, c_int, c_int, c_int, c_int, c_float, c_uint32, P, P, P, c_size_t, c_int, P]),
    "rlt_list_attention_bwd_prepare": (c_int, [P, P, P, c_int, c_int, c_int, c_int, c_float, P, P, c_size_t, c_int, P]),
    "rlt_list_attention_bwd_dkv": (c_int, [P, P, P, P, P, c_size_t, c_int, c_int, c_int, c_int, c_float, c_uint32, P, c_int, P]),
    "rlt_list_attention_bwd_dq": (c_int, [P, P, P, P, P, c_size_t, c_int, c_int, c_int, c_int, c_float, c_uint32, P, c_int, P]),
    "rlt_list_attention_plan": (c_int, [c_int, c_int, c_int, c_int, c_float, c_int, c_int, P]),
    "rlt_bilstm_rec_fwd": (c_int, [P, P, P, c_int, c_int, P, P, c_int, P]),
    "rlt_bilstm_rec_fwd_x": (c_int, [P, c_int, P, P, P, P, P, P, P, P, c_int, c_int, P, P, P, c_int, P]),
    "rlt_bilstm_rec_bwd": (c_int, [P, P, P, P, P, c_int, c_int, c_int, P]),
    "rlt_bilstm_rec_plan": (c_int, [c_int, c_int, c_int, P]),
    "rlt_to_position_major": (c_int, [P, c_int, c_int, c_int, P, P]),
    "rlt_from_position_major": (c_int, [P, c_int, c_int, c_int, P, P]),
    "rlt_choopy_embed": (c_int, [P, P, c_int, c_int, c_int, P, P]),
    "rlt_heads_fwd": (c_int, [P, P, P, P, c_int, c_int, c_int, c_int, P, P]),
    "rlt_heads_bwd_workspace": (c_size_t, [c_int, c_int, c_int, c_int]),
    "rlt_heads_bwd": (c_int, [P, P, P, c_int, P, P, c_int, c_int, c_int, P, c_int, P, P, P, c_size_t, P]),
    "rlt_mmoe_gate_fwd": (c_int, [P, P, c_int, c_int, c_int, c_int, c_int, P, P]),
    "rlt_mmoe_gate_bwd_workspace": (c_size_t, [c_int, c_int, c_int, c_int, c_int]),
    "rlt_mmoe_gate_bwd": (c_int, [P, P, P, P, c_int, c_int, c_int, c_int, c_int, P, c_int, P, P, c_size_t, P]),
    "rlt_mmoe_mix_fwd": (c_int, [P, P, c_int, c_int, c_int, c_int, c_int, P, P]),
    "rlt_mmoe_mix_bwd": (c_int, [P, P, P, c_int, c_int, c_int, c_int, c_int, P, P, P]),
    "rlt_adam_step": (c_int, [P, P, P, P, c_size_t, c_int, c_float, c_float, c_float, c_float, c_float, P]),
    "rlt_grad_norm_chunk": (c_size_t, []),
    "rlt_grad_norm_grid": (c_int, []),
    "rlt_grad_norm_workspace": (c_size_t, [c_size_t, c_int]),
    "rlt_grad_norm": (c_int, [P, c_size_t, P, c_int, c_float, P, c_size_t, P, P, P]),
    "rlt_adam_step_guarded": (c_int, [P, P, P, P, c_size_t, P, c_float, c_float, c_float, c_float, c_float, c_int, P]),
    "rlt_paired_compare_plan": (c_int, [c_int, c_int, c_int, P]),
    "rlt_paired_compare_workspace": (c_size_t, [c_int, c_int, c_int]),
    "rlt_paired_compare": (c_int, [P, P, c_int, c_int, c_int, c_int, c_uint32, P, c_size_t, P, P, P, P]),
    "rlt_workspace_bytes": (c_size_t, [c_int, c_int, c_int, c_int, c_int, c_int, c_int, c_int]),
    "rlt_encoder_layer_fwd": (c_int, [P, P, c_int, c_int, c_int, c_int, c_int, c_float, c_float, P, P, P, c_size_t, P, c_size_t, c_int, P]),
    "rlt_encoder_layer_bwd": (c_int, [P, P, c_int, c_int, c_int, c_int, c_int, c_float, c_float, P, P, P, c_size_t, P, P, P, c_size_t, c_int, P]),
    "rlt_bilstm_fwd": (c_int, [P, c_int, P, c_int, c_int, P, P, c_size_t, P, c_size_t, c_int, P]),
    "rlt_bilstm_bwd": (c_int, [P, c_int, P, P, P, c_int, c_int, P, c_size_t, P, P, P, c_size_t, c_int, P]),
    "rlt_sparse_inproj_workspace": (c_size_t, [c_int, c_int, c_int, c_int, c_int, c_int]),
    "rlt_sparse_inproj_fwd": (c_int, [P, c_int, c_int, P, P, P, P, P, P, P, P]),
    "rlt_sparse_inproj_bwd": (c_int, [P, c_int, c_int, P, P, P, P, P, P, P, P, c_size_t, P]),
    "rlt_bilstm_sparse_workspace": (c_size_t, [c_int, c_int, c_int, c_int, c_int, c_int]),
    "rlt_bilstm_sparse_fwd": (c_int, [P, P, c_int, c_int, P, P, c_size_t, P, c_size_t, c_int, P]),
    "rlt_bilstm_sparse_bwd": (c_int, [P, P, P, P, c_int, c_int, P, c_size_t, P, P, c_size_t, c_int, P]),
    "rlt_bilstm_generic_bytes": (c_size_t, [c_int, c_int, c_int, c_int, c_int]),
    "rlt_bilstm_generic_fwd": (c_int, [P, c_int, c_int, P, c_int, c_int, P, P, c_size_t, P, c_size_t, c_int, P]),
    "rlt_bilstm_generic_bwd": (c_int, [P, c_int, c_int, P, P, P, c_int, c_int, P, c_size_t, P, P, P, c_size_t, c_int, P]),
}
OP_ENCODER_STASH, OP_ENCODER_FWD_WS, OP_ENCODER_BWD_WS, OP_BILSTM_STASH, OP_BILSTM_WS = 1, 2, 3, 4, 5
ENCODER_FIELDS = ("in_proj_weight", "in_proj_bias", "out_proj_weight", "out_proj_bias", "norm1_weight", "norm1_bias",
                  "linear1_weight", "linear1_bias", "linear2_weight", "linear2_bias", "norm2_weight", "norm2_bias")


class EncoderPtrs(ctypes.Structure):
    _fields_ = [(f, c_void_p) for f in ENCODER_FIELDS]


class LstmLayerPtrs(ctypes.Structure):
    _fields_ = [("w_ih", c_void_p * 2), ("w_hh", c_void_p * 2), ("b_ih", c_void_p * 2), ("b_hh", c_void_p * 2)]


SPARSE_CHUNK = 256
SPARSE_POINTERS = ("dense", "ids", "perm", "indptr", "indices", "values", "col_ptr", "col_rows", "col_vals",
                   "chunk_col", "chunk_ptr", "multi_cols")
SPARSE_INTS = ("Dn", "n_docs", "V", "n_chunks", "n_multi")


class SparseBatchPtrs(ctypes.Structure):
    _fields_ = [(f, c_void_p) for f in SPARSE_POINTERS] + [(f, c_int) for f in SPARSE_INTS]


GEMM_FAMILIES = ("none", "gemm", "gemm3", "gemm3b", "gemm6", "gemm6b", "gemm6c", "gemm6e", "gemm6s")
GEMM_DISPATCH_FIELDS = ("family", "ta", "tb", "fast", "persistent", "ns", "kchunk", "slab_xcd", "epilogue", "narrow")


class GemmDispatch(ctypes.Structure):
    _fields_ = [(f, c_int) for f in GEMM_DISPATCH_FIELDS]


def gemm_last_dispatch():
    d = GemmDispatch()
    check(load().rlt_gemm_last_dispatch(ctypes.byref(d)), "rlt_gemm_last_dispatch")
    out = {f: int(getattr(d, f)) for f in GEMM_DISPATCH_FIELDS}
    out["family"] = GEMM_FAMILIES[out["family"]]
    return out


ATTN_KERNELS = ("none", "f32", "f32_sb", "f32_occ1", "f32_hd16", "x3", "x6", "x6_img", "x6_pp", "x6_pp_img", "x6_dkv1", "x6_dq1",
                "x6n_2w", "x6n_2w_seeded", "x6n_pipe", "x6h_pipe")
ATTN_PREPARE = ("q", "k", "v", "do", "seeds", "delta")
ATTN_IMAGES = ("none", "x3_qkv", "x6_qkv", "x6n_kv", "x6h_kv")
ATTN_WS = ("delta", "x3_do", "x6_do", "x6n_blocks")
ATTN_PLAN_INTS = ("fwd", "fwd_fixup", "dkv", "dq", "fwd_prepare", "bwd_prepare", "dkv_prepare", "dq_prepare",
                  "images_kind", "images_retained", "ws_kind")
ATTN_PLAN_SIZES = ("images_bytes", "flags_offset", "flags_bytes", "delta_bytes", "ws_extra_bytes", "ws_bytes",
                   "ws_prepare_bytes", "ws_part_bytes")


class AttentionPlan(ctypes.Structure):
    _fields_ = [(f, c_int) for f in ATTN_PLAN_INTS] + [(f, c_size_t) for f in ATTN_PLAN_SIZES]


def attention_plan(S, B, H, HD, drop_p, have_images, precision=PRECISION_DEFAULT):
    d = AttentionPlan()
    check(load().rlt_list_attention_plan(S, B, H, HD, drop_p, int(bool(have_images)), precision, ctypes.byref(d)), "rlt_list_attention_plan")
    out = {f: int(getattr(d, f)) for f in ATTN_PLAN_INTS + ATTN_PLAN_SIZES}
    for f in ("fwd", "fwd_fixup", "dkv", "dq"):
        out[f] = ATTN_KERNELS[out[f]]
    for f in ("fwd_prepare", "bwd_prepare", "dkv_prepare", "dq_prepare"):
        out[f] = tuple(n for i, n in enumerate(ATTN_PREPARE) if out[f] >> i & 1)
    out["images_kind"] = ATTN_IMAGES[out["images_kind"]]
    out["ws_kind"] = ATTN_WS[out["ws_kind"]]
    return out


LSTM_KERNELS = ("none", "f32", "x3", "x6", "x6w_single", "x6w_halves")
LSTM_PLAN_FIELDS = ("fwd", "bwd", "fwd_lists", "bwd_lists")


class BilstmRecPlan(ctypes.Structure):
    _fields_ = [(f, c_int) for f in LSTM_PLAN_FIELDS]


def bilstm_rec_plan(B, xin, precision=PRECISION_DEFAULT):
    d = BilstmRecPlan()
    check(load().rlt_bilstm_rec_plan(B, int(bool(xin)), precision, ctypes.byref(d)), "rlt_bilstm_rec_plan")
    out = {f: int(getattr(d, f)) for f in LSTM_PLAN_FIELDS}
    out["fwd"], out["bwd"] = LSTM_KERNELS[out["fwd"]], LSTM_KERNELS[out["bwd"]]
    return out


OPT_STATE_WORDS = 13
OPT_STEP, OPT_SKIPPED, OPT_CLIPPED, OPT_NONFINITE, OPT_NAN = 0, 1, 2, 3, 4
OPT_SUMSQ, OPT_NORM, OPT_MAX_ABS, OPT_NORM_SUM, OPT_NORM_MAX, OPT_NORM_STEPS = 5, 6, 7, 8, 9, 10
OPT_COEF_F32 = 22
GRAD_SEG_WORDS = 3


CMP_WORDS = 16
(CMP_N, CMP_SUM_BASE, CMP_SUM_SYS, CMP_SUM_D, CMP_SSD, CMP_WINS, CMP_TIES, CMP_LOSSES, CMP_NONFINITE, CMP_T_OBS, CMP_RAND_GE,
# ... 120 lines not shown
```

ranked-list-truncation_amd/rlt_hip/ops.py:

```python
import contextvars
import math

import torch
from torch.autograd import Function

from . import native as N
from .native import call, ptr, query, stream, workspace


def _empty(shape, like):
    return torch.empty(shape, dtype=torch.float32, device=like.device)


class KernelTimer:
    active = None

    def __init__(self):
        self.events = {}

    def reset(self):
        self.events = {}

    def timed(self, name, fn):
        a, b = torch.cuda.Event(enable_timing=True), torch.cuda.Event(enable_timing=True)
        a.record()
        fn()
        b.record()
        self.events.setdefault(name, []).append((a, b))

    def summary(self):
        return {k: (len(v), sum(a.elapsed_time(b) for a, b in v) / len(v)) for k, v in self.events.items()}


_SEED_COUNTER = [0]
_SEED_STREAM = [0]
KERNEL_LEVEL_ENCODER = [False]


def set_seed_stream(stream_id):
    _SEED_STREAM[0] = int(stream_id)


def next_seed():
    _SEED_COUNTER[0] += 1
    x = (torch.initial_seed() * 0x9E3779B97F4A7C15 + _SEED_COUNTER[0] * 0xD1B54A32D192ED03
         + _SEED_STREAM[0] * 0xA24BAED4963EE407) & 0xFFFFFFFFFFFFFFFF
    x ^= x >> 29
    return int((x * 0xBF58476D1CE4E5B9 >> 32) & 0xFFFFFFFF)


_CALL_PRECISION = contextvars.ContextVar("rlt_call_precision", default=N.PRECISION_DEFAULT)


class precision:

    def __init__(self, mode):
        self.code = N.PRECISION_DEFAULT if mode is None else N.precision_code(mode)
        self._tokens = []

    def __enter__(self):
        self._tokens.append(_CALL_PRECISION.set(self.code))
        return self

    def __exit__(self, *exc):
        _CALL_PRECISION.reset(self._tokens.pop())
        return False


def current_precision():
    c = _CALL_PRECISION.get()
    return c if c >= 0 else int(N.load().rlt_get_precision())


def _launch(name, fn):
    t = KernelTimer.active
    if t is None:
        fn()
    else:
        t.timed(name, fn)


def gemm(ta, tb, M, Nn, K, A, lda, B, ldb, C, ldc, bias=None, bias2=None, flags=0, a_off=0, b_off=0, c_off=0,
         relu_mask=None, ldmask=0, colsum_a=None, mask_scale=1.0, drop_p=0.0, seed=0, prec=None):
    ws_bytes = query("rlt_gemm_workspace", ta, tb, M, Nn, K)
    ws = workspace(ws_bytes, C.device) if ws_bytes else None
    esz = 4
    call("rlt_gemm_ex", ta, tb, M, Nn, K,
         N.c_void_p(A.data_ptr() + a_off * esz), lda, N.c_void_p(B.data_ptr() + b_off * esz), ldb,
         N.c_void_p(C.data_ptr() + c_off * esz), ldc, ptr(bias), ptr(bias2), flags,
         ptr(relu_mask), ldmask, mask_scale, ptr(colsum_a), drop_p, seed, ptr(ws), ws_bytes,
         current_precision() if prec is None else prec, stream())


def gemm_bits(ta, tb, M, Nn, K, A, lda, B, ldb, C, ldc, bias=None, flags=0, bits_out=None, bits_in=None, mask_scale=1.0,
              drop_p=0.0, seed=0, prec=None):
    call("rlt_gemm_bits", ta, tb, M, Nn, K, ptr(A), lda, ptr(B), ldb, ptr(C), ldc, ptr(bias), flags, drop_p, seed,
         ptr(bits_out), ptr(bits_in), mask_scale, current_precision() if prec is None else prec, stream())


def alloc_relu_bits(M, Nn, device):
    return torch.zeros(((M + 31) // 32, Nn), dtype=torch.int32, device=device)


def unpack_relu_bits(bits, M):
    sh = torch.arange(32, dtype=torch.int32, device=bits.device).view(1, 32, 1)
    return (((bits.unsqueeze(1) >> sh) & 1).reshape(-1, bits.shape[1])[:M]).bool()


def colsum(X, ldx, T, Nn, out, accumulate=0, x_off=0):
    ws_bytes = query("rlt_colsum_workspace", T, Nn)
    ws = workspace(ws_bytes, X.device)
    call("rlt_colsum", N.c_void_p(X.data_ptr() + 4 * x_off), ldx, T, Nn, ptr(out), accumulate, ptr(ws), ws_bytes, stream())


class LinearFn(Function):

    @staticmethod
    def forward(ctx, x, w, b, relu):
        T, K = x.shape
        Nn = w.shape[0]
        y = _empty((T, Nn), x)
        ctx.prec = current_precision()
        gemm(0, 1, T, Nn, K, x, K, w, K, y, Nn, bias=b, flags=N.GEMM_RELU if relu else 0, prec=ctx.prec)
        ctx.relu = relu
        ctx.save_for_backward(x, w, y if relu else None)
        return y

    @staticmethod
    def backward(ctx, dy):
        x, w, y = ctx.saved_tensors
        T, K = x.shape
        Nn = w.shape[0]
        dy = N.f32c(dy)
        if ctx.relu:
            dy = dy.clone()
            call("rlt_relu_bwd", ptr(dy), ptr(y), dy.numel(), stream())
        dx = dw = db = None
        if ctx.needs_input_grad[0]:
            dx = _empty((T, K), x)
            gemm(0, 0, T, K, Nn, dy, Nn, w, K, dx, K, prec=ctx.prec)
        if ctx.needs_input_grad[1]:
            dw = _empty((Nn, K), x)
            db = _empty((Nn,), x) if ctx.needs_input_grad[2] else None
            gemm(1, 0, Nn, K, T, dy, Nn, x, K, dw, K, colsum_a=db, prec=ctx.prec)
        elif ctx.needs_input_grad[2]:
            db = _empty((Nn,), x)
            colsum(dy, Nn, T, Nn, db)
        return dx, dw, db, None


def linear(x, w, b, relu=False):
    return LinearFn.apply(x, w, b, relu)


class FFNFn(Function):

    @staticmethod
    def forward(ctx, x, w1, b1, w2, b2, drop_p=0.0, seed=0):
        T, E = x.shape
        Fh = w1.shape[0]
        h = _empty((T, Fh), x)
        ctx.prec = pr = current_precision()
        gemm(0, 1, T, Fh, E, x, E, w1, E, h, Fh, bias=b1, flags=N.GEMM_RELU, drop_p=drop_p, seed=seed, prec=pr)
        y = _empty((T, w2.shape[0]), x)
        gemm(0, 1, T, w2.shape[0], Fh, h, Fh, w2, Fh, y, w2.shape[0], bias=b2, prec=pr)
        ctx.save_for_backward(x, w1, w2, h)
        ctx.drop_p = drop_p
        return y

    @staticmethod
    def backward(ctx, dy):
        x, w1, w2, h = ctx.saved_tensors
        T, E = x.shape
        Fh, Eo = w1.shape[0], w2.shape[0]
        dy = N.f32c(dy)
        pr = ctx.prec
        dw2, db2 = _empty((Eo, Fh), x), _empty((Eo,), x)
        gemm(1, 0, Eo, Fh, T, dy, Eo, h, Fh, dw2, Fh, colsum_a=db2, prec=pr)
        dh = _empty((T, Fh), x)
        gemm(0, 0, T, Fh, Eo, dy, Eo, w2, Fh, dh, Fh, relu_mask=h, ldmask=Fh, mask_scale=1.0 / (1.0 - ctx.drop_p), prec=pr)
        dw1, db1 = _empty((Fh, E), x), _empty((Fh,), x)
        gemm(1, 0, Fh, E, T, dh, Fh, x, E, dw1, E, colsum_a=db1, prec=pr)
        dx = None
        if ctx.needs_input_grad[0]:
            dx = _empty((T, E), x)
            gemm(0, 0, T, E, Fh, dh, Fh, w1, E, dx, E, prec=pr)
        return dx, dw1, db1, dw2, db2, None, None


def ffn(x, w1, b1, w2, b2, drop_p=0.0):
    return FFNFn.apply(x, w1, b1, w2, b2, drop_p, next_seed() if drop_p > 0 else 0)


class AddLayerNormFn(Function):
    @staticmethod
    def forward(ctx, x, r, gamma, beta, eps, drop_p=0.0, seed=0):
        T, E = x.shape
        y = _empty((T, E), x)
        stats = _empty((T, 2), x)
        call("rlt_add_layernorm_fwd", ptr(x), ptr(r), ptr(gamma), ptr(beta), T, E, eps, drop_p, seed,
             ptr(y), ptr(stats), stream())
        ctx.save_for_backward(x, r, gamma, stats)
        ctx.drop = (drop_p, seed)
        return y

    @staticmethod
    def backward(ctx, dy):
        x, r, gamma, stats = ctx.saved_tensors
        T, E = x.shape
        dy = N.f32c(dy)
        drop_p, seed = ctx.drop
        dz = _empty((T, E), x)
        dr = _empty((T, E), x) if drop_p > 0 else None
        dgamma, dbeta = _empty((E,), x), _empty((E,), x)
        ws_bytes = query("rlt_add_layernorm_bwd_workspace", T, E)
        ws = workspace(ws_bytes, x.device)
        call("rlt_add_layernorm_bwd", ptr(x), ptr(r), ptr(gamma), ptr(stats), ptr(dy), T, E, drop_p, seed,
             ptr(dz), ptr(dr), ptr(dgamma), ptr(dbeta), 0, ptr(ws), ws_bytes, stream())
        return dz, (dz if dr is None else dr), dgamma, dbeta, None, None, None


def add_layernorm(x, r, gamma, beta, eps=1e-5, drop_p=0.0):
    return AddLayerNormFn.apply(x, r, gamma, beta, eps, drop_p, next_seed() if drop_p > 0 else 0)


class ListAttentionFn(Function):

    @staticmethod
    def forward(ctx, qkv, S, B, H, drop_p=0.0, seed=0):
        E = qkv.shape[1] // 3
        HD = E // H
        out = _empty((S * B, E), qkv)
        lse = _empty((S, H, B), qkv)
        ctx.prec = pr = current_precision()
        img_bytes = query("rlt_list_attention_fwd_workspace", S, B, H, HD, drop_p, pr)
        images = workspace(img_bytes, qkv.device) if img_bytes else None
        _launch("attn_fwd", lambda: call("rlt_list_attention_fwd", ptr(qkv), S, B, H, HD, drop_p, seed,
                                         ptr(out), ptr(lse), ptr(images), img_bytes, pr, stream()))
        ctx.dims = (S, B, H, HD)
        ctx.drop = (drop_p, seed)
        ctx.images = images if images is not None and N.load().rlt_list_attention_images_retained(S, B, H, HD, pr) else None
        ctx.save_for_backward(qkv, out, lse)
        return out

    @staticmethod
    def backward(ctx, dout):
        qkv, out, lse = ctx.saved_tensors
        S, B, H, HD = ctx.dims
        images = ctx.images
        dout = N.f32c(dout)
        dqkv = torch.empty_like(qkv)
        pr = ctx.prec
        drop_p, seed = ctx.drop
        ws_bytes = query("rlt_list_attention_bwd_workspace", S, B, H, HD, drop_p, pr)
        ws = workspace(ws_bytes, qkv.device)
        call("rlt_list_attention_bwd_prepare", ptr(out), ptr(dout), ptr(lse), S, B, H, HD, drop_p, ptr(images), ptr(ws), ws_bytes, pr, stream())
        _launch("attn_bwd_dkv", lambda: call("rlt_list_attention_bwd_dkv", ptr(qkv), ptr(dout), ptr(lse), ptr(images), ptr(ws), ws_bytes,
                                             S, B, H, HD, drop_p, seed, ptr(dqkv), pr, stream()))
        _launch("attn_bwd_dq", lambda: call("rlt_list_attention_bwd_dq", ptr(qkv), ptr(dout), ptr(lse), ptr(images), ptr(ws), ws_bytes,
                                            S, B, H, HD, drop_p, seed, ptr(dqkv), pr, stream()))
        ctx.images = None
        return dqkv, None, None, None, None, None


def list_attention(qkv, S, B, H, drop_p=0.0):
    return ListAttentionFn.apply(qkv, S, B, H, drop_p, next_seed() if drop_p > 0 else 0)


class EncoderLayerFn(Function):

    @staticmethod
    def forward(ctx, x, in_w, in_b, out_w, out_b, n1_w, n1_b, w1, b1, w2, b2, n2_w, n2_b, S, B, H, eps, drop_p, seeds):
        T, E = x.shape
        FF = w1.shape[0]
        if T != S * B or in_w.shape != (3 * E, E) or w2.shape != (E, FF):
            raise RuntimeError(f"encoder layer: x {tuple(x.shape)} does not match S*B = {S * B} / the layer's weights")
        weights = (in_w, in_b, out_w, out_b, n1_w, n1_b, w1, b1, w2, b2, n2_w, n2_b)
        pr = current_precision()
        stash_bytes = query("rlt_workspace_bytes", N.OP_ENCODER_STASH, S, B, E, H, FF, 0, pr)
        ws_bytes = query("rlt_workspace_bytes", N.OP_ENCODER_FWD_WS, S, B, E, H, FF, 1 if drop_p > 0 else 0, pr)
        stash = N.byte_buffer(stash_bytes, x.device)
        ws = N.byte_buffer(ws_bytes, x.device)
        y = _empty((T, E), x)
        sarr = (N.c_uint32 * 4)(*seeds)
        wp = N.encoder_ptrs(weights)
        _launch("encoder_fwd", lambda: call("rlt_encoder_layer_fwd", ptr(x), N.ctypes.byref(wp), S, B, E, H, FF, eps, drop_p, sarr,
                                            ptr(y), ptr(stash), stash_bytes, ptr(ws), ws_bytes, pr, stream()))
        ctx.cfg = (S, B, E, H, FF, eps, drop_p, tuple(seeds), stash_bytes, pr)
        ctx.stash = stash
        ctx.save_for_backward(x, *weights)
        return y

    @staticmethod
    def backward(ctx, dy):
        x, *weights = ctx.saved_tensors
        S, B, E, H, FF, eps, drop_p, seeds, stash_bytes, pr = ctx.cfg
        if ctx.stash is None:
            raise RuntimeError("EncoderLayerFn.backward frees its stash and can run only once")
        dy = N.f32c(dy)
        dx = torch.empty_like(x)
        grads = [torch.empty_like(w) for w in weights]
        ws_bytes = query("rlt_workspace_bytes", N.OP_ENCODER_BWD_WS, S, B, E, H, FF, 1 if drop_p > 0 else 0, pr)
        ws = N.byte_buffer(ws_bytes, x.device)
        sarr = (N.c_uint32 * 4)(*seeds)
        wp, gp = N.encoder_ptrs(weights), N.encoder_ptrs(grads)
        _launch("encoder_bwd", lambda: call("rlt_encoder_layer_bwd", ptr(x), N.ctypes.byref(wp), S, B, E, H, FF, eps, drop_p, sarr,
                                            ptr(dy), ptr(ctx.stash), stash_bytes, ptr(dx), N.ctypes.byref(gp),
                                            ptr(ws), ws_bytes, pr, stream()))
        ctx.stash = None
        return (dx, *grads, None, None, None, None, None, None)


class EncoderLayerKernelsFn(Function):

    @staticmethod
    def forward(ctx, *args):
        ctx.prec = current_precision()
        with precision(ctx.prec):
            return EncoderLayerKernelsFn._forward(ctx, *args)

    @staticmethod
    def backward(ctx, dy):
        with precision(ctx.prec):
            return EncoderLayerKernelsFn._backward(ctx, dy)

    @staticmethod
    def _forward(ctx, x, in_w, in_b, out_w, out_b, n1_w, n1_b, w1, b1, w2, b2, n2_w, n2_b, S, B, H, eps, drop_p, seeds):
        T, E = x.shape
        HD = E // H
        Fh = w1.shape[0]
        pr = ctx.prec
        s_attn, s_ln1, s_ffn, s_ln2 = seeds
        qkv = _empty((T, 3 * E), x)
        gemm(0, 1, T, 3 * E, E, x, E, in_w, E, qkv, 3 * E, bias=in_b)
        att = _empty((T, E), x)
        lse = _empty((S, H, B), x)
        img_bytes = query("rlt_list_attention_fwd_workspace", S, B, H, HD, drop_p, pr)
        images = workspace(img_bytes, x.device) if img_bytes else None
        _launch("attn_fwd", lambda: call("rlt_list_attention_fwd", ptr(qkv), S, B, H, HD, drop_p, s_attn,
                                         ptr(att), ptr(lse), ptr(images), img_bytes, pr, stream()))
        if images is not None and not N.load().rlt_list_attention_images_retained(S, B, H, HD, pr):
            images = None
        proj = _empty((T, E), x)
        gemm(0, 1, T, E, E, att, E, out_w, E, proj, E, bias=out_b)
        h1 = _empty((T, E), x)
        st1 = _empty((T, 2), x)
        call("rlt_add_layernorm_fwd", ptr(x), ptr(proj), ptr(n1_w), ptr(n1_b), T, E, eps, drop_p, s_ln1, ptr(h1), ptr(st1), stream())
        hid = _empty((T, Fh), x)
        relu_bits = None
        if Fh % 32 == 0:
            relu_bits = alloc_relu_bits(T, Fh, x.device)
            gemm_bits(0, 1, T, Fh, E, h1, E, w1, E, hid, Fh, bias=b1, flags=N.GEMM_RELU, bits_out=relu_bits,
                      drop_p=drop_p, seed=s_ffn)
        else:
            gemm(0, 1, T, Fh, E, h1, E, w1, E, hid, Fh, bias=b1, flags=N.GEMM_RELU, drop_p=drop_p, seed=s_ffn)
        ff = _empty((T, E), x)
        gemm(0, 1, T, E, Fh, hid, Fh, w2, Fh, ff, E, bias=b2)
        y = _empty((T, E), x)
        st2 = _empty((T, 2), x)
        call("rlt_add_layernorm_fwd", ptr(h1), ptr(ff), ptr(n2_w), ptr(n2_b), T, E, eps, drop_p, s_ln2, ptr(y), ptr(st2), stream())
        ctx.cfg = (S, B, H, HD, eps, drop_p, seeds)
        ctx.images = images
        ctx.relu_bits = relu_bits
        ctx.save_for_backward(x, in_w, out_w, n1_w, w1, w2, n2_w, qkv, att, lse, proj, st1, h1, hid, ff, st2)
        return y

    @staticmethod
    def _backward(ctx, dy):
        x, in_w, out_w, n1_w, w1, w2, n2_w, qkv, att, lse, proj, st1, h1, hid, ff, st2 = ctx.saved_tensors
        S, B, H, HD, eps, drop_p, (s_attn, s_ln1, s_ffn, s_ln2) = ctx.cfg
        pr = ctx.prec
        T, E = x.shape
        Fh = w1.shape[0]
        dy = N.f32c(dy)

        def ln_bwd(xx, rr, gamma, stats, dyy, seed):
            dz = _empty((T, E), x)
            dr = _empty((T, E), x) if drop_p > 0 else None
            dg, db = _empty((E,), x), _empty((E,), x)
            ws_bytes = query("rlt_add_layernorm_bwd_workspace", T, E)
            ws = workspace(ws_bytes, x.device)
            call("rlt_add_layernorm_bwd", ptr(xx), ptr(rr), ptr(gamma), ptr(stats), ptr(dyy), T, E, drop_p, seed,
                 ptr(dz), ptr(dr), ptr(dg), ptr(db), 0, ptr(ws), ws_bytes, stream())
            return dz, (dz if dr is None else dr), dg, db

        dz2, dr2, dn2_w, dn2_b = ln_bwd(h1, ff, n2_w, st2, dy, s_ln2)
        dw2, db2 = _empty((E, Fh), x), _empty((E,), x)
        gemm(1, 0, E, Fh, T, dr2, E, hid, Fh, dw2, Fh, colsum_a=db2)
        dhid = _empty((T, Fh), x)
        if ctx.relu_bits is not None:
            gemm_bits(0, 0, T, Fh, E, dr2, E, w2, Fh, dhid, Fh, bits_in=ctx.relu_bits, mask_scale=1.0 / (1.0 - drop_p))
            ctx.relu_bits = None
        else:
            gemm(0, 0, T, Fh, E, dr2, E, w2, Fh, dhid, Fh, relu_mask=hid, ldmask=Fh, mask_scale=1.0 / (1.0 - drop_p))
        dw1, db1 = _empty((Fh, E), x), _empty((Fh,), x)
        gemm(1, 0, Fh, E, T, dhid, Fh, h1, E, dw1, E, colsum_a=db1)
        gemm(0, 0, T, E, Fh, dhid, Fh, w1, E, dz2, E, flags=N.GEMM_ACCUMULATE)
        del dhid
        dz1, dr1, dn1_w, dn1_b = ln_bwd(x, proj, n1_w, st1, dz2, s_ln1)
        dw_o, db_o = _empty((E, E), x), _empty((E,), x)
        gemm(1, 0, E, E, T, dr1, E, att, E, dw_o, E, colsum_a=db_o)
        datt = _empty((T, E), x)
        gemm(0, 0, T, E, E, dr1, E, out_w, E, datt, E)
        images = ctx.images
        dqkv = torch.empty_like(qkv)
        ws_bytes = query("rlt_list_attention_bwd_workspace", S, B, H, HD, drop_p, pr)
        ws = workspace(ws_bytes, x.device)
        call("rlt_list_attention_bwd_prepare", ptr(att), ptr(datt), ptr(lse), S, B, H, HD, drop_p, ptr(images), ptr(ws), ws_bytes, pr, stream())
        _launch("attn_bwd_dkv", lambda: call("rlt_list_attention_bwd_dkv", ptr(qkv), ptr(datt), ptr(lse), ptr(images), ptr(ws), ws_bytes,
                                             S, B, H, HD, drop_p, s_attn, ptr(dqkv), pr, stream()))
        _launch("attn_bwd_dq", lambda: call("rlt_list_attention_bwd_dq", ptr(qkv), ptr(datt), ptr(lse), ptr(images), ptr(ws), ws_bytes,
                                            S, B, H, HD, drop_p, s_attn, ptr(dqkv), pr, stream()))
        ctx.images = None
        dw_in, db_in = _empty((3 * E, E), x), _empty((3 * E,), x)
        gemm(1, 0, 3 * E, E, T, dqkv, 3 * E, x, E, dw_in, E, colsum_a=db_in)
        gemm(0, 0, T, E, 3 * E, dqkv, 3 * E, in_w, E, dz1, E, flags=N.GEMM_ACCUMULATE)
        return (dz1, dw_in, db_in, dw_o, db_o, dn1_w, dn1_b, dw1, db1, dw2, db2, dn2_w, dn2_b,
                None, None, None, None, None, None)


def encoder_layer(x, layer, S, B, H, drop_p=0.0, eps=1e-5):
    att = layer.self_attn
    seeds = tuple(next_seed() for _ in range(4)) if drop_p > 0 else (0, 0, 0, 0)
    fn = EncoderLayerKernelsFn if (KernelTimer.active is not None or KERNEL_LEVEL_ENCODER[0]) else EncoderLayerFn
    return fn.apply(x, att.in_proj_weight, att.in_proj_bias, att.out_proj.weight, att.out_proj.bias,
                                layer.norm1.weight, layer.norm1.bias, layer.linear1.weight, layer.linear1.bias,
                                layer.linear2.weight, layer.linear2.bias, layer.norm2.weight, layer.norm2.bias,
                                S, B, H, eps, drop_p, seeds)


def encoder_ffn_hidden(y):
    node = y.grad_fn if torch.is_tensor(y) else y
    if type(node).__name__ != "EncoderLayerFnBackward" or node.stash is None:
        raise RuntimeError("not the output of a live encoder-layer tape node")
    S, B, E, H, FF = node.cfg[:5]
    T, rup = S * B, lambda n: (n + 255) // 256 * 256
    off = rup(T * 3 * E * 4) + rup(T * E * 4) + rup(S * H * B * 4) + rup(T * E * 4) + rup(T * 2 * 4) + rup(T * E * 4)
    return node.stash[off:off + T * FF * 4].view(torch.float32).view(T, FF)


class BiLSTMFn(Function):

    @staticmethod
    def forward(ctx, x, S, B, *w):
        T, I = x.shape
        if len(w) != 16:
            raise RuntimeError("BiLSTMFn takes the 16 parameters of a 2-layer bidirectional LSTM")
        Hd = w[1].shape[1]
        if w[0].shape != (4 * Hd, I) or w[4].shape != (4 * Hd, I) or w[8].shape != (4 * Hd, 2 * Hd) or w[1].shape != (4 * Hd, Hd) or T != S * B:
            raise RuntimeError(f"BiLSTM input has {I} features x {T} rows; the layers were built for "
                               f"{w[0].shape[1]} features, hidden {Hd} and S*B = {S * B} rows")
        fast = Hd == 128
        pr = current_precision()
        if fast:
            stash_bytes = query("rlt_workspace_bytes", N.OP_BILSTM_STASH, S, B, I, 0, 0, 0, pr)
            ws_bytes = query("rlt_workspace_bytes", N.OP_BILSTM_WS, S, B, I, 0, 0, 0, pr)
        else:
            stash_bytes = query("rlt_bilstm_generic_bytes", 1, S, B, I, Hd)
            ws_bytes = query("rlt_bilstm_generic_bytes", 0, S, B, I, Hd)
        stash = N.byte_buffer(stash_bytes, x.device)
        ws = N.byte_buffer(ws_bytes, x.device)
        h = _empty((T, 2 * Hd), x)
        wp = N.lstm_ptrs([w[0:8], w[8:16]])
        if fast:
            _launch("bilstm_fwd", lambda: call("rlt_bilstm_fwd", ptr(x), I, wp, S, B, ptr(h), ptr(stash), stash_bytes,
                                               ptr(ws), ws_bytes, pr, stream()))
        else:
            call("rlt_bilstm_generic_fwd", ptr(x), I, Hd, wp, S, B, ptr(h), ptr(stash), stash_bytes, ptr(ws), ws_bytes, pr, stream())
        ctx.cfg = (S, B, I, Hd, stash_bytes, ws_bytes, pr)
        ctx.stash = stash
        ctx.save_for_backward(x, h, *w)
        return h

    @staticmethod
    def backward(ctx, dh):
        if ctx.stash is None:
            raise RuntimeError("BiLSTMFn.backward overwrites its stash in place and can run only once")
        x, h, *w = ctx.saved_tensors
        S, B, I, Hd, stash_bytes, ws_bytes, pr = ctx.cfg
        dh = N.f32c(dh)
        grads = [torch.empty_like(t) for t in w]
        dx = torch.empty_like(x) if ctx.needs_input_grad[0] else None
        ws = N.byte_buffer(ws_bytes, x.device)
        wp, gp = N.lstm_ptrs([w[0:8], w[8:16]]), N.lstm_ptrs([grads[0:8], grads[8:16]])
        if Hd == 128:
            _launch("bilstm_bwd", lambda: call("rlt_bilstm_bwd", ptr(x), I, wp, ptr(h), ptr(dh), S, B, ptr(ctx.stash), stash_bytes,
                                               ptr(dx), gp, ptr(ws), ws_bytes, pr, stream()))
        else:
            call("rlt_bilstm_generic_bwd", ptr(x), I, Hd, wp, ptr(h), ptr(dh), S, B, ptr(ctx.stash), stash_bytes,
                 ptr(dx), gp, ptr(ws), ws_bytes, pr, stream())
        ctx.stash = None
        return (dx, None, None, *grads)


def bilstm(x, params, S, B):
    names = ("weight_ih", "weight_hh", "bias_ih", "bias_hh")
    w = [getattr(params, f"{n}_l{layer}{suffix}") for layer in (0, 1) for suffix in ("", "_reverse") for n in names]
    return BiLSTMFn.apply(x, S, B, *w)


class SparseBatch:

    def __init__(self, dense, ids, table, validate=False):
        if dense.dim() != 3 or dense.dtype != torch.float32 or ids.dim() != 2 or ids.dtype != torch.int32 \
                or tuple(dense.shape[:2]) != tuple(ids.shape):
            raise ValueError("SparseBatch: dense must be (B, S, Dn) float32 and ids (B, S) int32 over the same lists")
        if not 1 <= dense.shape[2] <= 16:
            raise ValueError(f"SparseBatch: {dense.shape[2]} dense columns; the kernels take 1..16")
        self.dense, self.ids, self.table, self.validate = dense, ids, table, validate

    @property
    def shape(self):
        return (self.ids.shape[0], self.ids.shape[1], self.dense.shape[2] + int(self.table.V))

    def __getitem__(self, lists):
        if not isinstance(lists, slice):
            raise TypeError("SparseBatch: index with a slice of lists")
        return SparseBatch(self.dense[lists], self.ids[lists], self.table, self.validate)

    def to_dense(self):
        B, S, Dn = self.dense.shape
        t = self.table
        x = torch.zeros((B * S, Dn + int(t.V)), dtype=torch.float32, device=self.ids.device)
        x[:, :Dn] = self.dense.reshape(B * S, Dn)
        ids = self.ids.reshape(-1).long()
        n = (t.indptr[ids + 1] - t.indptr[ids])
        rows = torch.repeat_interleave(torch.arange(B * S, device=ids.device), n)
        pos = torch.arange(int(n.sum()), device=ids.device) - torch.repeat_interleave(torch.cumsum(n, 0) - n, n)
        j = torch.repeat_interleave(t.indptr[ids], n) + pos
        x[rows, Dn + t.indices[j].long()] = t.values[j]
        return x.view(B, S, -1)

    def struct(self, perm=None):
        t = self.table
        dense = self.dense if self.dense.is_contiguous() else self.dense.contiguous()
        ids = self.ids if self.ids.is_contiguous() else self.ids.contiguous()
        N.require_cuda(dense, ids, t.indptr, t.indices, t.values, t.col_ptr, t.col_rows, t.col_vals, t.chunk_col, t.chunk_ptr, t.multi_cols)
        if t.indptr.dtype != torch.int64 or t.indices.dtype != torch.int32 or t.values.dtype != torch.float32 \
                or t.indptr.numel() != int(t.n_docs) + 1 or t.col_ptr.dtype != torch.int64 or t.col_ptr.numel() != int(t.V) + 1 \
                or t.chunk_ptr.numel() != int(t.V) + 1 or t.chunk_col.numel() != int(t.n_chunks):
            raise ValueError("SparseBatch: the table's arrays must be indptr (n_docs+1) int64, indices int32, values float32 and "
                             "the term index of dataloader.bicut_data.term_index")
        if self.validate:
            lo, hi = torch.aminmax(ids)
            if int(lo) < 0 or int(hi) >= int(t.n_docs):
                raise ValueError(f"SparseBatch: document row outside [0, {int(t.n_docs)}): min {int(lo)}, max {int(hi)}")
        keep = (dense, ids, perm)
        sb = N.SparseBatchPtrs()
        for name, a in (("dense", dense), ("ids", ids), ("perm", perm)):
            setattr(sb, name, None if a is None else a.data_ptr())
        for name in N.SPARSE_POINTERS[3:]:
            setattr(sb, name, getattr(t, name).data_ptr())
        sb.Dn, sb.n_docs, sb.V, sb.n_chunks, sb.n_multi = dense.shape[2], int(t.n_docs), int(t.V), int(t.n_chunks), int(t.n_multi)
        return sb, keep


class BiLSTMSparseFn(Function):

    @staticmethod
    def forward(ctx, batch, S, B, *w):
        if len(w) != 16:
            raise RuntimeError("BiLSTMSparseFn takes the 16 parameters of a 2-layer bidirectional LSTM")
        I = batch.shape[2]
        for k in (0, 4):
            if tuple(w[k].shape) != (512, I) or w[k].stride() != (1, 512):
                raise RuntimeError(f"sparse BiLSTM: layer-0 input weight of shape {tuple(w[k].shape)} and strides {w[k].stride()}; "
                                   f"the batch needs (512, {I}) stored column-major, strides (1, 512)")
        if tuple(batch.ids.shape) != (B, S) or tuple(w[1].shape) != (512, 128) or tuple(w[8].shape) != (512, 256):
            raise RuntimeError("sparse BiLSTM: hidden size 128, two layers, ids (B, S)")
# ... 604 lines not shown
```

Baseline: 24710 lists/s.

## Pre-split weight operand into bf16x3 LDS image for 6-product GEMMs

Adds a kernel that converts a weight matrix once into a pre-swizzled hi/mid/lo bf16 image laid out to match the GEMM's LDS tiles. A new GEMM variant streams that image straight into shared memory instead of loading fp32 B and splitting it in every workgroup. This is wired into the encoder's weight-operand GEMMs (FFN linear2 forward, linear1 and in_proj data-gradient backward, LSTM dx) when K is at least 1024. It removes the redundant per-tile B split arithmetic and VGPR pressure, but adds an image-build launch per call, 1.5x the B memory traffic, and extra workspace.

```diff
diff --git a/include/rlt_hip.h b/include/rlt_hip.h
--- a/include/rlt_hip.h
+++ b/include/rlt_hip.h
@@ -105,6 +105,17 @@
     int family, ta, tb, fast, persistent, ns, kchunk, slab_xcd, epilogue, narrow;
 } rlt_gemm_dispatch;
 int rlt_gemm_last_dispatch(rlt_gemm_dispatch* out);
+
+size_t rlt_gemm_wimage_bytes(int tb, int N, int K);
+int rlt_gemm_wimage(int tb, int N, int K, const float* B, int ldb, void* image, size_t image_bytes, void* stream);
+int rlt_gemm_bimg(int ta, int tb, int M, int N, int K,
+                  const float* A, int lda, const float* B, int ldb, float* C, int ldc,
+                  const float* bias, const float* bias2, int flags,
+                  const void* b_image, size_t b_image_bytes,
+                  void* ws, size_t ws_bytes, int precision, void* stream);
+int rlt_gemm_last_b_image(void);
+int rlt_gemm_wimage_enabled(void);
+int rlt_gemm_bimg_hint(int ta, int tb, int M, int N, int K, int precision);
 
 size_t rlt_gemm_bits_words(int M, int N);
 int rlt_gemm_bits(int ta, int tb, int M, int N, int K,
diff --git a/ranked-list-truncation_amd/csrc/gemm.hip b/ranked-list-truncation_amd/csrc/gemm.hip
--- a/ranked-list-truncation_amd/csrc/gemm.hip
+++ b/ranked-list-truncation_amd/csrc/gemm.hip
@@ -27,6 +27,7 @@
     uint32_t* bits_out;
     const uint32_t* bits_in;
     int ldbits;
+    const uint16_t* bimg;
 };
 
 inline void note_dispatch(int family, bool ta, bool tb, bool fast, bool persistent, const GemmArgs& g, int ns) {
@@ -1446,8 +1447,30 @@
     return !g.mask && !g.bits_in && !g.bits_out && g.drop_p <= 0.f;
 }
 
-template <bool TA, bool TB, bool PERSIST>
-__global__ __launch_bounds__(256, 1) void gemm6e_kernel(GemmArgs g) {
+
+constexpr int WIMG6 = 3 * HB6;
+typedef unsigned int u32x4 __attribute__((ext_vector_type(4)));
+__global__ __launch_bounds__(256) void gemm_wimage_kernel(const float* __restrict__ W, int ld, int tb, int K, uint16_t* __restrict__ img) {
+    const int ks = blockIdx.x, np = blockIdx.y, n = threadIdx.x;
+    const int pr = phys6(n);
+    uint16_t* blk = img + ((size_t)np * (K >> 4) + ks) * WIMG6;
+    const float* src = tb ? W + (size_t)(np * 256 + n) * ld + 16 * ks : W + (size_t)(16 * ks) * ld + np * 256 + n;
+    const size_t kstride = tb ? 1 : (size_t)ld;
+#pragma unroll
+    for (int x = 0; x < 4; ++x) {
+        const float a = src[(4 * x) * kstride], b = src[(4 * x + 1) * kstride], c = src[(4 * x + 2) * kstride], d = src[(4 * x + 3) * kstride];
+        Split6 su;
+#pragma unroll
+        for (int part = 0; part < 6; ++part) split6_part(su, a, b, c, d, part);
+        uint16_t* dst = blk + pr * 16 + 8 * ((x >> 1) ^ ((pr >> 3) & 1)) + 4 * (x & 1);
+        *reinterpret_cast<uint2*>(dst) = su.hi;
+        *reinterpret_cast<uint2*>(dst + HB6) = su.mid;
+        *reinterpret_cast<uint2*>(dst + 2 * HB6) = su.lo;
+    }
+}
+
+template <bool TA, bool TB, bool PERSIST, bool BIMG>
+__device__ __forceinline__ void gemm6e_body(const GemmArgs& g) {
     extern __shared__ __attribute__((aligned(16))) float gsm[];
     uint16_t* lds = reinterpret_cast<uint16_t*>(gsm);
     const int tid = threadIdx.x, lane = tid & 63, wv = __builtin_amdgcn_readfirstlane(tid >> 6);
@@ -1503,7 +1526,21 @@
         const int k0 = kbeg + 16 * (wrap ? ks - nks : min(ks, nks - 1)), nn = wrap ? nn0 : n0;
         return g.B + (BKC ? (size_t)nn * g.ldb + k0 : (size_t)k0 * g.ldb + nn) + offB;
     };
+    auto srcI = [&](int ks) {
+        const bool wrap = PERSIST && has_next && ks >= nks;
+        const int k0 = kbeg + 16 * (wrap ? ks - nks : min(ks, nks - 1)), nn = wrap ? nn0 : n0;
+        return reinterpret_cast<const u32x4*>(g.bimg + ((size_t)(nn >> 8) * (g.K >> 4) + (k0 >> 4)) * WIMG6) + tid;
+    };
     float4 ra[2][4], rb[2][4];
+    u32x4 ri[2][6];
+    auto load_img = [&](const u32x4* pi, u32x4 (&v)[6]) {
+#pragma unroll
+        for (int n = 0; n < 6; ++n) v[n] = pi[256 * n];
+    };
+    auto stash_img = [&](uint16_t* wb, const u32x4 (&v)[6]) {
+#pragma unroll
+        for (int n = 0; n < 6; ++n) *reinterpret_cast<u32x4*>(wb + 3 * HB6 + 8 * (tid + 256 * n)) = v[n];
+    };
     auto add_cs = [&](const float4 (&v)[4]) {
 #pragma unroll
         for (int i = 0; i < 4; ++i) { csum.x += v[i].x; csum.y += v[i].y; csum.z += v[i].z; csum.w += v[i].w; }
@@ -1518,18 +1555,43 @@
             *reinterpret_cast<uint2*>(wb + dA[p]) = hi;
             *reinterpret_cast<uint2*>(wb + dA[p] + HB6) = mid;
             *reinterpret_cast<uint2*>(wb + dA[p] + 2 * HB6) = lo;
-            vals6e<BKC>(vb, p, a, b, c, d);
-            split4x3(a, b, c, d, hi, mid, lo);
-            *reinterpret_cast<uint2*>(wb + dB[p]) = hi;
-            *reinterpret_cast<uint2*>(wb + dB[p] + HB6) = mid;
-            *reinterpret_cast<uint2*>(wb + dB[p] + 2 * HB6) = lo;
+            if (!BIMG) {
+                vals6e<BKC>(vb, p, a, b, c, d);
+                split4x3(a, b, c, d, hi, mid, lo);
+                *reinterpret_cast<uint2*>(wb + dB[p]) = hi;
+                *reinterpret_cast<uint2*>(wb + dB[p] + HB6) = mid;
+                *reinterpret_cast<uint2*>(wb + dB[p] + 2 * HB6) = lo;
+            }
         }
     };
     bf16x8 a[4][3], b[2][3];
     auto frag_a = [&](const uint16_t* base, int i, int q) { a[i][q] = *reinterpret_cast<const bf16x8*>(base + arow + q * HB6 + i * 32 * 16); };
     auto frag_b = [&](const uint16_t* base, int j, int q) { b[j & 1][q] = *reinterpret_cast<const bf16x8*>(base + brow + q * HB6 + j * 32 * 16); };
 
-    {
+    if constexpr (BIMG) {
+        const float* pa = srcA(0);
+#pragma unroll
+        for (int i = 0; i < 4; ++i) load6e<AKC>(pa, g.lda, i, ra[0][i]);
+        load_img(srcI(0), ri[0]);
+        pa = srcA(1);
+#pragma unroll
+        for (int i = 0; i < 4; ++i) load6e<AKC>(pa, g.lda, i, ra[1][i]);
+        load_img(srcI(1), ri[1]);
+        if (want_cs) { add_cs(ra[0]); add_cs(ra[1]); }
+        stash_all(lds, ra[0], rb[0]);
+        stash_img(lds, ri[0]);
+        stash_all(lds + KB6, ra[1], rb[1]);
+        stash_img(lds + KB6, ri[1]);
+        if (PERSIST) decode_next();
+        pa = srcA(2);
+#pragma unroll
+        for (int i = 0; i < 4; ++i) load6e<AKC>(pa, g.lda, i, ra[0][i]);
+        load_img(srcI(2), ri[0]);
+        pa = srcA(3);
+#pragma unroll
+        for (int i = 0; i < 4; ++i) load6e<AKC>(pa, g.lda, i, ra[1][i]);
+        load_img(srcI(3), ri[1]);
+    } else {
         const float* pa = srcA(0); const float* pb = srcB(0);
 #pragma unroll
         for (int i = 0; i < 4; ++i) { load6e<AKC>(pa, g.lda, i, ra[0][i]); load6e<BKC>(pb, g.ldb, i, rb[0][i]); }
@@ -1551,7 +1613,7 @@
 #pragma unroll
     for (int q = 0; q < 3; ++q) { frag_a(lds, 0, q); frag_a(lds, 1, q); frag_b(lds, 0, q); }
 
-    auto slot = [&](auto par_tag, int buf, int wbuf, int nbuf, const float* pa, const float* pb) {
+    auto slot = [&](auto par_tag, int buf, int wbuf, int nbuf, const float* pa, const float* pb, const u32x4* pi) {
         constexpr int PAR = decltype(par_tag)::value;
         const uint16_t* base = lds + buf * KB6;
         const uint16_t* nbase = lds + nbuf * KB6;
@@ -1572,7 +1634,13 @@
                    else if ((p_) == 7) { for (int i_ = 0; i_ < 4; ++i_) load6e<BKC>(pb, g.ldb, i_, rb[PAR][i_]); } } } while (0)
 #define RA(i_, q_, n_) frag_a((n_) ? nbase : base, i_, q_)
 #define RB(j_, q_, n_) frag_b((n_) ? nbase : base, j_, q_)
+#define IB(n_) do { *reinterpret_cast<u32x4*>(wb + 3 * HB6 + 8 * (tid + 256 * (n_))) = ri[PAR][n_]; ri[PAR][n_] = pi[256 * (n_)]; } while (0)
+        if constexpr (BIMG) {
+#include "gemm6e_slot_bimg.inc"
+        } else {
 #include "gemm6e_slot.inc"
+        }
+#undef IB
 #undef GAP_END
 #undef MM
 #undef SP
@@ -1586,10 +1654,10 @@
         for (int s = 0; s < nks; s += 2) {
             const int u1 = u == 2 ? 0 : u + 1, u2 = u1 == 2 ? 0 : u1 + 1;
             if (want_cs && s + 2 < nks) add_cs(ra[0]);
-            slot(std::integral_constant<int, 0>{}, u, u2, u1, srcA(s + 4), srcB(s + 4));
+            slot(std::integral_constant<int, 0>{}, u, u2, u1, srcA(s + 4), BIMG ? nullptr : srcB(s + 4), BIMG ? srcI(s + 4) : nullptr);
             __syncthreads();
             if (want_cs && s + 3 < nks) add_cs(ra[1]);
-            slot(std::integral_constant<int, 1>{}, u1, u, u2, srcA(s + 5), srcB(s + 5));
+            slot(std::integral_constant<int, 1>{}, u1, u, u2, srcA(s + 5), BIMG ? nullptr : srcB(s + 5), BIMG ? srcI(s + 5) : nullptr);
             __syncthreads();
             u = u2;
         }
@@ -1621,6 +1689,31 @@
             dst[0] = t.x; dst[1] = t.y; dst[2] = t.z; dst[3] = t.w;
         }
     }
+}
+template <bool TA, bool TB, bool PERSIST>
+__global__ __launch_bounds__(256, 1) void gemm6e_kernel(GemmArgs g) { gemm6e_body<TA, TB, PERSIST, false>(g); }
+template <bool TB, bool PERSIST>
+__global__ __launch_bounds__(256, 1) void gemm6e_bimg_kernel(GemmArgs g) { gemm6e_body<false, TB, PERSIST, true>(g); }
+
+template <bool TB>
+int launch_gemm6e_bimg(GemmArgs g, int ns, hipStream_t st) {
+    const size_t shm = (size_t)3 * KB6 * sizeof(uint16_t);
+    g.tiles_m = g.M / BM2; g.tiles_n = g.N / BN2;
+    static const int persist_wgs = [] { const char* e = getenv("RLT_GEMM6_PERSIST"); return e ? atoi(e) : 256; }();
+    const long long tiles = (long long)g.tiles_m * g.tiles_n;
+    if (persist_wgs > 0 && ns == 1 && tiles > persist_wgs && persist_wgs % 8 == 0) {
+        int rc = rlt_allow_lds(gemm6e_bimg_kernel<TB, true>, shm);
+        if (rc) return rc;
+        note_dispatch(RLT_GEMM_6E, false, TB, true, true, g, ns);
+        hipLaunchKernelGGL((gemm6e_bimg_kernel<TB, true>), dim3(persist_wgs), dim3(256), shm, st, g);
+        return RLT_LAUNCH_RESULT();
+    }
+    int rc = rlt_allow_lds(gemm6e_bimg_kernel<TB, false>, shm);
+    if (rc) return rc;
+    dim3 grid(g.tiles_m * g.tiles_n * (g.slab_xcd ? ns : 1), 1, g.slab_xcd ? 1 : ns);
+    note_dispatch(RLT_GEMM_6E, false, TB, true, false, g, ns);
+    hipLaunchKernelGGL((gemm6e_bimg_kernel<TB, false>), grid, dim3(256), shm, st, g);
+    return RLT_LAUNCH_RESULT();
 }
 template <bool TA, bool TB>
 int launch_gemm6e(GemmArgs g, int ns, hipStream_t st) {
@@ -1873,6 +1966,12 @@
 }
 
 thread_local rlt_gemm_dispatch rlt_gemm_dispatch_rec = {};
+static thread_local int gemm_bimg_rec = 0;
+
+static bool wimg_on() {
+    static const bool on = [] { const char* e = getenv("RLT_GEMM_WIMG"); return !e || atoi(e) != 0; }();
+    return on;
+}
 
 extern "C" {
 
@@ -1903,8 +2002,9 @@
                     const float* bias, const float* bias2, int flags,
                     const float* relu_mask, int ldmask, float mask_scale, float* colsum_a,
                     float drop_p, uint32_t seed, uint32_t* bits_out, const uint32_t* bits_in,
-                    void* ws, size_t ws_bytes, void* stream) {
+                    void* ws, size_t ws_bytes, void* stream, const void* b_image = nullptr) {
     rlt_gemm_dispatch_rec = rlt_gemm_dispatch{};
+    gemm_bimg_rec = 0;
     RLT_CHECK_ARG(A && B && C && M > 0 && N > 0 && K > 0);
     RLT_CHECK_ARG(lda >= (ta ? M : K) && ldb >= (tb ? K : N) && ldc >= N);
     RLT_CHECK_ARG(!relu_mask || ldmask >= N);
@@ -1915,6 +2015,7 @@
     g.bits_out = bits_out; g.bits_in = bits_in; g.ldbits = N;
     g.mask_scale = mask_scale; g.drop_p = drop_p; g.drop_thr = rlt_drop_threshold(drop_p); g.seed = seed;
     g.A = A; g.B = B; g.C = C; g.bias = bias; g.bias2 = bias2;
+    g.bimg = wimg_on() ? static_cast<const uint16_t*>(b_image) : nullptr;
     g.M = M; g.N = N; g.K = K; g.lda = lda; g.ldb = ldb; g.ldc = ldc;
     g.vecA = (lda % 4 == 0) && rlt_aligned16(A);
     g.vecB = (ldb % 4 == 0) && rlt_aligned16(B);
@@ -1949,7 +2050,10 @@
         static const bool x6_e = [] { const char* e = getenv("RLT_GEMM6E"); return !e || atoi(e) != 0; }();
         static const bool x6_e_all = [] { const char* e = getenv("RLT_GEMM6E_ALL"); return e && atoi(e) != 0; }();
         if (x6_e && gemm6e_epilogue_ok(g) && (ta || g.K >= 1024 || x6_e_all)) {
-            if (!ta && tb) rc = launch_gemm6e<false, true>(g, ns, st);
+            if (!ta && g.bimg) {
+                gemm_bimg_rec = 1;
+                rc = tb ? launch_gemm6e_bimg<true>(g, ns, st) : launch_gemm6e_bimg<false>(g, ns, st);
+            } else if (!ta && tb) rc = launch_gemm6e<false, true>(g, ns, st);
             else if (!ta && !tb) rc = launch_gemm6e<false, false>(g, ns, st);
             else if (!tb) rc = launch_gemm6e<true, false>(g, ns, st);
             else rc = launch_gemm6e<true, true>(g, ns, st);
@@ -2000,6 +2104,47 @@
                     drop_p, seed, nullptr, nullptr, ws, ws_bytes, stream);
 }
 
+size_t rlt_gemm_wimage_bytes(int tb, int N, int K) {
+    (void)tb;
+    if (N <= 0 || K <= 0 || N % BN2 || K % BK3) return 0;
+    return (size_t)N * (size_t)K * 3 * sizeof(uint16_t);
+}
+
+int rlt_gemm_wimage(int tb, int N, int K, const float* B, int ldb, void* image, size_t image_bytes, void* stream) {
+    RLT_CHECK_ARG(B && image && N > 0 && K > 0 && ldb >= (tb ? K : N));
+    const size_t need = rlt_gemm_wimage_bytes(tb, N, K);
+    RLT_CHECK_SHAPE(need > 0);
+    if (image_bytes < need) return RLT_E_WORKSPACE;
+    RLT_CHECK_ARG(rlt_aligned16(image));
+    hipLaunchKernelGGL(gemm_wimage_kernel, dim3(K / 16, N / BN2), dim3(256), 0, rlt_stream(stream), B, ldb, tb ? 1 : 0, K,
+                       static_cast<uint16_t*>(image));
+    return RLT_LAUNCH_RESULT();
+}
+
+int rlt_gemm_wimage_enabled(void) { return wimg_on() ? 1 : 0; }
+
+int rlt_gemm_last_b_image(void) { return gemm_bimg_rec; }
+
+int rlt_gemm_bimg_hint(int ta, int tb, int M, int N, int K, int precision) {
+    RLT_PREC_SCOPE_SZ(precision);
+    if (!wimg_on() || gemm_mode() != 2 || ta || !rlt_gemm_wimage_bytes(tb, N, K) || M <= 0 || M % BM2 || K < 1024) return 0;
+    int ns = choose_split(M, N, K);
+    const int kchunk = rlt_cdiv(rlt_cdiv(K, ns), 32) * 32;
+    return kchunk / BK3 >= 2 && (K % kchunk == 0 || (K % kchunk) / BK3 >= 2);
+}
+
+int rlt_gemm_bimg(int ta, int tb, int M, int N, int K,
+                  const float* A, int lda, const float* B, int ldb, float* C, int ldc,
+                  const float* bias, const float* bias2, int flags,
+                  const void* b_image, size_t b_image_bytes,
+                  void* ws, size_t ws_bytes, int precision, void* stream) {
+    RLT_PREC_SCOPE(precision);
+    const size_t need = rlt_gemm_wimage_bytes(tb, N, K);
+    if (!b_image || !need || b_image_bytes < need || !rlt_aligned16(b_image)) b_image = nullptr;
+    return gemm_run(ta, tb, M, N, K, A, lda, B, ldb, C, ldc, bias, bias2, flags, nullptr, 0, 1.0f, nullptr,
+                    0.0f, 0u, nullptr, nullptr, ws, ws_bytes, stream, b_image);
+}
+
 size_t rlt_gemm_bits_words(int M, int N) { return M > 0 && N > 0 ? (size_t)rlt_cdiv(M, 32) * N : 0; }
 
 int rlt_gemm_bits(int ta, int tb, int M, int N, int K,
diff --git a/ranked-list-truncation_amd/csrc/gemm6e_slot_bimg.inc b/ranked-list-truncation_amd/csrc/gemm6e_slot_bimg.inc
--- /dev/null
+++ b/ranked-list-truncation_amd/csrc/gemm6e_slot_bimg.inc
@@ -0,0 +1,96 @@
+MM(0, 0, 0); GAP_END; SP(0, 0); GAP_END;
+MM(0, 0, 1); GAP_END; SP(0, 1); GAP_END;
+MM(0, 0, 2); GAP_END; SP(0, 2); GAP_END;
+MM(0, 0, 3); GAP_END; SP(0, 3); GAP_END;
+MM(0, 0, 4); GAP_END; SP(0, 4); GAP_END;
+MM(0, 0, 5); GAP_END; SP(0, 5); RA(2, 0, 0); GAP_END;
+MM(1, 0, 0); GAP_END; ST(0); GAP_END;
+MM(1, 0, 1); GAP_END; RA(2, 1, 0); RA(2, 2, 0); GAP_END;
+MM(1, 0, 2); GAP_END; RA(3, 0, 0); RA(3, 1, 0); GAP_END;
+MM(1, 0, 3); GAP_END; RA(3, 2, 0); RB(1, 0, 0); GAP_END;
+MM(1, 0, 4); GAP_END; RB(1, 1, 0); RB(1, 2, 0); GAP_END;
+MM(1, 0, 5); GAP_END; GAP_END;
+MM(2, 0, 0); GAP_END; SP(1, 0); GAP_END;
+MM(2, 0, 1); GAP_END; SP(1, 1); GAP_END;
+MM(2, 0, 2); GAP_END; SP(1, 2); GAP_END;
+MM(2, 0, 3); GAP_END; SP(1, 3); GAP_END;
+MM(2, 0, 4); GAP_END; SP(1, 4); GAP_END;
+MM(2, 0, 5); GAP_END; SP(1, 5); GAP_END;
+MM(3, 0, 0); GAP_END; ST(1); GAP_END;
+MM(3, 0, 1); GAP_END; GAP_END;
+MM(3, 0, 2); GAP_END; GAP_END;
+MM(3, 0, 3); GAP_END; GAP_END;
+MM(3, 0, 4); GAP_END; GAP_END;
+MM(3, 0, 5); GAP_END; GAP_END;
+MM(0, 1, 0); GAP_END; SP(2, 0); GAP_END;
+MM(0, 1, 1); GAP_END; SP(2, 1); GAP_END;
+MM(0, 1, 2); GAP_END; SP(2, 2); GAP_END;
+MM(0, 1, 3); GAP_END; SP(2, 3); GAP_END;
+MM(0, 1, 4); GAP_END; SP(2, 4); GAP_END;
+MM(0, 1, 5); GAP_END; SP(2, 5); RB(2, 0, 0); GAP_END;
+MM(1, 1, 0); GAP_END; ST(2); GAP_END;
+MM(1, 1, 1); GAP_END; RB(2, 1, 0); RB(2, 2, 0); GAP_END;
+MM(1, 1, 2); GAP_END; GAP_END;
+MM(1, 1, 3); GAP_END; GAP_END;
+MM(1, 1, 4); GAP_END; GAP_END;
+MM(1, 1, 5); GAP_END; GAP_END;
+MM(2, 1, 0); GAP_END; SP(3, 0); GAP_END;
+MM(2, 1, 1); GAP_END; SP(3, 1); GAP_END;
+MM(2, 1, 2); GAP_END; SP(3, 2); GAP_END;
+MM(2, 1, 3); GAP_END; SP(3, 3); GAP_END;
+MM(2, 1, 4); GAP_END; SP(3, 4); GAP_END;
+MM(2, 1, 5); GAP_END; SP(3, 5); GAP_END;
+MM(3, 1, 0); GAP_END; ST(3); GAP_END;
+MM(3, 1, 1); GAP_END; GAP_END;
+MM(3, 1, 2); GAP_END; GAP_END;
+MM(3, 1, 3); GAP_END; GAP_END;
+MM(3, 1, 4); GAP_END; GAP_END;
+MM(3, 1, 5); GAP_END; GAP_END;
+MM(0, 2, 0); GAP_END; IB(0); GAP_END;
+MM(0, 2, 1); GAP_END; RB(3, 0, 0); RB(3, 1, 0); GAP_END;
+MM(0, 2, 2); GAP_END; RB(3, 2, 0); GAP_END;
+MM(0, 2, 3); GAP_END; GAP_END;
+MM(0, 2, 4); GAP_END; GAP_END;
+MM(0, 2, 5); GAP_END; GAP_END;
+MM(1, 2, 0); GAP_END; IB(1); GAP_END;
+MM(1, 2, 1); GAP_END; GAP_END;
+MM(1, 2, 2); GAP_END; GAP_END;
+MM(1, 2, 3); GAP_END; GAP_END;
+MM(1, 2, 4); GAP_END; GAP_END;
+MM(1, 2, 5); GAP_END; GAP_END;
+MM(2, 2, 0); GAP_END; IB(2); GAP_END;
+MM(2, 2, 1); GAP_END; GAP_END;
+MM(2, 2, 2); GAP_END; GAP_END;
+MM(2, 2, 3); GAP_END; GAP_END;
+MM(2, 2, 4); GAP_END; GAP_END;
+MM(2, 2, 5); GAP_END; GAP_END;
+MM(3, 2, 0); GAP_END; IB(3); GAP_END;
+MM(3, 2, 1); GAP_END; GAP_END;
+MM(3, 2, 2); GAP_END; GAP_END;
+MM(3, 2, 3); GAP_END; GAP_END;
+MM(3, 2, 4); GAP_END; GAP_END;
+MM(3, 2, 5); GAP_END; GAP_END;
+MM(0, 3, 0); GAP_END; IB(4); GAP_END;
+MM(0, 3, 1); GAP_END; RB(0, 0, 1); RB(0, 1, 1); GAP_END;
+MM(0, 3, 2); GAP_END; RB(0, 2, 1); GAP_END;
+MM(0, 3, 3); GAP_END; GAP_END;
+MM(0, 3, 4); GAP_END; GAP_END;
+MM(0, 3, 5); GAP_END; GAP_END;
+MM(1, 3, 0); GAP_END; IB(5); GAP_END;
+MM(1, 3, 1); GAP_END; RA(0, 0, 1); RA(0, 1, 1); GAP_END;
+MM(1, 3, 2); GAP_END; RA(0, 2, 1); GAP_END;
+MM(1, 3, 3); GAP_END; GAP_END;
+MM(1, 3, 4); GAP_END; GAP_END;
+MM(1, 3, 5); GAP_END; GAP_END;
+MM(2, 3, 0); GAP_END; RA(1, 0, 1); RA(1, 1, 1); GAP_END;
+MM(2, 3, 1); GAP_END; RA(1, 2, 1); GAP_END;
+MM(2, 3, 2); GAP_END; GAP_END;
+MM(2, 3, 3); GAP_END; GAP_END;
+MM(2, 3, 4); GAP_END; GAP_END;
+MM(2, 3, 5); GAP_END; GAP_END;
+MM(3, 3, 0); GAP_END; GAP_END;
+MM(3, 3, 1); GAP_END; GAP_END;
+MM(3, 3, 2); GAP_END; GAP_END;
+MM(3, 3, 3); GAP_END; GAP_END;
+MM(3, 3, 4); GAP_END; GAP_END;
+MM(3, 3, 5); GAP_END; GAP_END;
diff --git a/ranked-list-truncation_amd/csrc/path.hip b/ranked-list-truncation_amd/csrc/path.hip
--- a/ranked-list-truncation_amd/csrc/path.hip
+++ b/ranked-list-truncation_amd/csrc/path.hip
@@ -62,11 +62,16 @@
     if (rlt_list_attention_images_retained(d.S, d.B, d.H, d.HD, RLT_PRECISION_DEFAULT)) return 0;
     return rlt_list_attention_fwd_workspace(d.S, d.B, d.H, d.HD, drop_p, RLT_PRECISION_DEFAULT);
 }
+inline size_t enc_fwd_wimg(const EncDims& d) { return rlt_gemm_wimage_bytes(1, d.E, d.FF); }
+inline size_t enc_bwd_wimg(const EncDims& d) {
+    const size_t a = rlt_gemm_wimage_bytes(0, d.E, d.FF), b = rlt_gemm_wimage_bytes(0, d.E, 3 * d.E);
+    return a > b ? a : b;
+}
 
 struct EncScratch {
     float *dz2, *dr2, *dhid, *dr1, *datt, *dqkv;
-    void *attn_ws, *ln_ws, *gemm_ws;
-    size_t attn_ws_bytes, ln_ws_bytes, gemm_ws_bytes, bytes;
+    void *attn_ws, *ln_ws, *gemm_ws, *wimg;
+    size_t attn_ws_bytes, ln_ws_bytes, gemm_ws_bytes, wimg_bytes, bytes;
 };
 inline size_t enc_gemm_ws(const EncDims& d) {
     const int T = (int)d.T;
@@ -104,6 +109,8 @@
     w.ln_ws = c.take<uint8_t>(w.ln_ws_bytes);
     w.gemm_ws_bytes = enc_gemm_ws(d);
     w.gemm_ws = c.take<uint8_t>(w.gemm_ws_bytes);
+    w.wimg_bytes = enc_bwd_wimg(d);
+    w.wimg = w.wimg_bytes ? c.take<uint8_t>(w.wimg_bytes) : nullptr;
     w.bytes = c.off;
     return w;
 }
@@ -114,6 +121,15 @@
                 const float* bias, int flags, float* colsum_a, void* ws, size_t ws_bytes, void* st) {
     return rlt_gemm_ex(ta, tb, M, N, K, A, lda, B, ldb, C, ldc, bias, nullptr, flags, nullptr, 0, 1.f, colsum_a, 0.f, 0u,
                        ws, ws_bytes, RLT_PRECISION_DEFAULT, st);
+}
+
+inline int gemm_w(int tb, int M, int N, int K, const float* A, int lda, const float* B, int ldb, float* C, int ldc,
+                  const float* bias, int flags, void* wimg, size_t wimg_bytes, void* ws, size_t ws_bytes, void* st) {
+    const size_t need = rlt_gemm_wimage_bytes(tb, N, K);
+    const bool use = wimg && need && need <= wimg_bytes && rlt_gemm_bimg_hint(0, tb, M, N, K, RLT_PRECISION_DEFAULT);
+    if (use) RLT_TRY(rlt_gemm_wimage(tb, N, K, B, ldb, wimg, wimg_bytes, st));
+    return rlt_gemm_bimg(0, tb, M, N, K, A, lda, B, ldb, C, ldc, bias, nullptr, flags, use ? wimg : nullptr, use ? need : 0,
+                         ws, ws_bytes, RLT_PRECISION_DEFAULT, st);
 }
 
 struct LstmStash { float *gates[2], *c[2], *h0; size_t bytes; };
@@ -128,7 +144,7 @@
     s.bytes = cur.off;
     return s;
 }
-struct LstmScratch { float *wcat, *bcat, *dh0, *dwcat, *dbcat; void* ws; size_t ws_bytes, bytes; };
+struct LstmScratch { float *wcat, *bcat, *dh0, *dwcat, *dbcat; void* ws; size_t ws_bytes; void* wimg; size_t wimg_bytes, bytes; };
 inline LstmScratch lstm_scratch(size_t T, int I, void* base, size_t cap = (size_t)-1) {
     Cursor cur(base, cap);
     LstmScratch w{};
@@ -146,6 +162,8 @@
     up(rlt_gemm_workspace(0, 0, (int)T, Imax, 1024));
     w.ws_bytes = m;
     w.ws = cur.take<uint8_t>(m);
+    w.wimg_bytes = rlt_gemm_wimage_bytes(0, 256, 1024);
+    w.wimg = cur.take<uint8_t>(w.wimg_bytes);
     w.bytes = cur.off;
     return w;
 }
@@ -221,7 +239,7 @@
     }
     if (dx) {
         RLT_TRY(pack2(w.w_ih[0], w.w_ih[1], (size_t)512 * I, sc.wcat, st));
-        RLT_TRY(gemm(0, 0, T, I, 1024, dA, 1024, sc.wcat, I, dx, I, nullptr, 0, nullptr, sc.ws, sc.ws_bytes, stream));
+        RLT_TRY(gemm_w(0, T, I, 1024, dA, 1024, sc.wcat, I, dx, I, nullptr, 0, sc.wimg, sc.wimg_bytes, sc.ws, sc.ws_bytes, stream));
     }
     return 0;
 }
@@ -247,7 +265,8 @@
         EncDims d;
         if (enc_dims(S, B, E, H, FF, d)) return 0;
         if (op == RLT_OP_ENCODER_STASH) return enc_stash(d, nullptr).bytes;
-        if (op == RLT_OP_ENCODER_FWD_WS) return rup(enc_gemm_ws(d)) + rup(enc_fwd_images_scratch(d, train_dropout ? 0.5f : 0.f));
+        if (op == RLT_OP_ENCODER_FWD_WS)
+            return rup(enc_gemm_ws(d)) + rup(enc_fwd_images_scratch(d, train_dropout ? 0.5f : 0.f)) + rup(enc_fwd_wimg(d));
         return enc_scratch(d, train_dropout != 0, nullptr).bytes;
     }
     if (op == RLT_OP_BILSTM_STASH || op == RLT_OP_BILSTM_WS) {
@@ -272,6 +291,8 @@
     if (stash_bytes < enc_stash(d, nullptr).bytes || ws_bytes < gemm_ws + img_scratch || (gemm_ws + img_scratch && !ws)) return RLT_E_WORKSPACE;
     EncStash s = enc_stash(d, stash, stash_bytes);
     if (img_scratch) { s.images = static_cast<uint8_t*>(ws) + gemm_ws; s.images_bytes = img_scratch; }
+    const size_t wimg_off = gemm_ws + rup(img_scratch), wimg_bytes = enc_fwd_wimg(d);
+    void* wimg = (wimg_bytes && ws && ws_bytes >= wimg_off + wimg_bytes) ? static_cast<uint8_t*>(ws) + wimg_off : nullptr;
     const int T = (int)d.T;
     const uint32_t s_attn = drop_p > 0.f ? seeds[0] : 0u, s_ln1 = drop_p > 0.f ? seeds[1] : 0u,
                    s_ffn = drop_p > 0.f ? seeds[2] : 0u, s_ln2 = drop_p > 0.f ? seeds[3] : 0u;
@@ -286,7 +307,7 @@
         RLT_TRY(rlt_gemm_ex(0, 1, T, FF, E, s.h1, E, w->linear1_weight, E, s.hid, FF, w->linear1_bias, nullptr, RLT_GEMM_RELU,
                             nullptr, 0, 1.f, nullptr, drop_p, s_ffn, ws, ws_bytes, RLT_PRECISION_DEFAULT, stream));
     }
-    RLT_TRY(gemm(0, 1, T, E, FF, s.hid, FF, w->linear2_weight, FF, s.ff, E, w->linear2_bias, 0, nullptr, ws, ws_bytes, stream));
+    RLT_TRY(gemm_w(1, T, E, FF, s.hid, FF, w->linear2_weight, FF, s.ff, E, w->linear2_bias, 0, wimg, wimg_bytes, ws, ws_bytes, stream));
     return rlt_add_layernorm_fwd(s.h1, s.ff, w->norm2_weight, w->norm2_bias, T, E, eps, drop_p, s_ln2, y, s.st2, stream);
 }
 
@@ -320,7 +341,7 @@
                             nullptr, 0.f, 0u, k.gemm_ws, k.gemm_ws_bytes, RLT_PRECISION_DEFAULT, stream));
     }
     RLT_TRY(gemm(1, 0, FF, E, T, k.dhid, FF, s.h1, E, g->linear1_weight, E, nullptr, 0, g->linear1_bias, k.gemm_ws, k.gemm_ws_bytes, stream));
-    RLT_TRY(gemm(0, 0, T, E, FF, k.dhid, FF, w->linear1_weight, E, k.dz2, E, nullptr, RLT_GEMM_ACCUMULATE, nullptr, k.gemm_ws, k.gemm_ws_bytes, stream));
+    RLT_TRY(gemm_w(0, T, E, FF, k.dhid, FF, w->linear1_weight, E, k.dz2, E, nullptr, RLT_GEMM_ACCUMULATE, k.wimg, k.wimg_bytes, k.gemm_ws, k.gemm_ws_bytes, stream));
     RLT_TRY(rlt_add_layernorm_bwd(x, s.proj, w->norm1_weight, s.st1, k.dz2, T, E, drop_p, s_ln1, dx, k.dr1,
                                   g->norm1_weight, g->norm1_bias, 0, k.ln_ws, k.ln_ws_bytes, stream));
     const float* dr1 = drop ? k.dr1 : dx;
@@ -329,7 +350,7 @@
     RLT_TRY(rlt_list_attention_bwd(s.qkv, s.att, k.datt, s.lse, S, B, H, d.HD, drop_p, s_attn, s.images, k.dqkv,
                                    k.attn_ws, k.attn_ws_bytes, RLT_PRECISION_DEFAULT, stream));
     RLT_TRY(gemm(1, 0, 3 * E, E, T, k.dqkv, 3 * E, x, E, g->in_proj_weight, E, nullptr, 0, g->in_proj_bias, k.gemm_ws, k.gemm_ws_bytes, stream));
-    return gemm(0, 0, T, E, 3 * E, k.dqkv, 3 * E, w->in_proj_weight, E, dx, E, nullptr, RLT_GEMM_ACCUMULATE, nullptr, k.gemm_ws, k.gemm_ws_bytes, stream);
+    return gemm_w(0, T, E, 3 * E, k.dqkv, 3 * E, w->in_proj_weight, E, dx, E, nullptr, RLT_GEMM_ACCUMULATE, k.wimg, k.wimg_bytes, k.gemm_ws, k.gemm_ws_bytes, stream);
 }
 
 int rlt_bilstm_fwd(const float* x, int I, const rlt_lstm_layer_weights* w, int S, int B, float* h_out,
diff --git a/ranked-list-truncation_amd/rlt_hip/native.py b/ranked-list-truncation_amd/rlt_hip/native.py
--- a/ranked-list-truncation_amd/rlt_hip/native.py
+++ b/ranked-list-truncation_amd/rlt_hip/native.py
@@ -59,6 +59,13 @@
     "rlt_gemm_ex": (c_int, [c_int, c_int, c_int, c_int, c_int, P, c_int, P, c_int, P, c_int, P, P, c_int, P, c_int, c_float,
                             P, c_float, c_uint32, P, c_size_t, c_int, P]),
     "rlt_gemm_last_dispatch": (c_int, [P]),
+    "rlt_gemm_wimage_bytes": (c_size_t, [c_int, c_int, c_int]),
+    "rlt_gemm_wimage": (c_int, [c_int, c_int, c_int, P, c_int, P, c_size_t, P]),
+    "rlt_gemm_bimg": (c_int, [c_int, c_int, c_int, c_int, c_int, P, c_int, P, c_int, P, c_int, P, P, c_int, P, c_size_t,
+                              P, c_size_t, c_int, P]),
+    "rlt_gemm_last_b_image": (c_int, []),
+    "rlt_gemm_wimage_enabled": (c_int, []),
+    "rlt_gemm_bimg_hint": (c_int, [c_int, c_int, c_int, c_int, c_int, c_int]),
     "rlt_dropout_mask": (c_int, [c_uint32, c_size_t, c_int, c_float, P, P]),
     "rlt_attention_dropout_mask": (c_int, [c_uint32, c_int, c_int, c_int, c_float, P, P]),
     "rlt_attention_dropout_mask_range": (c_int, [c_uint32, c_int, c_int, c_int, c_float, P, P]),
diff --git a/ranked-list-truncation_amd/rlt_hip/ops.py b/ranked-list-truncation_amd/rlt_hip/ops.py
--- a/ranked-list-truncation_amd/rlt_hip/ops.py
+++ b/ranked-list-truncation_amd/rlt_hip/ops.py
@@ -90,6 +90,19 @@
          N.c_void_p(C.data_ptr() + c_off * esz), ldc, ptr(bias), ptr(bias2), flags,
          ptr(relu_mask), ldmask, mask_scale, ptr(colsum_a), drop_p, seed, ptr(ws), ws_bytes,
          current_precision() if prec is None else prec, stream())
+
+
+def gemm_w(tb, M, Nn, K, A, lda, B, ldb, C, ldc, bias=None, flags=0):
+    pr = current_precision()
+    need = query("rlt_gemm_wimage_bytes", tb, Nn, K)
+    if not need or not N.load().rlt_gemm_bimg_hint(0, tb, M, Nn, K, pr):
+        return gemm(0, tb, M, Nn, K, A, lda, B, ldb, C, ldc, bias=bias, flags=flags)
+    img = N.byte_buffer(need, C.device)
+    call("rlt_gemm_wimage", tb, Nn, K, ptr(B), ldb, ptr(img), need, stream())
+    ws_bytes = query("rlt_gemm_workspace", 0, tb, M, Nn, K)
+    ws = workspace(ws_bytes, C.device) if ws_bytes else None
+    call("rlt_gemm_bimg", 0, tb, M, Nn, K, ptr(A), lda, ptr(B), ldb, ptr(C), ldc, ptr(bias), None, flags, ptr(img), need,
+         ptr(ws), ws_bytes, pr, stream())
 
 
 def gemm_bits(ta, tb, M, Nn, K, A, lda, B, ldb, C, ldc, bias=None, flags=0, bits_out=None, bits_in=None, mask_scale=1.0,
@@ -355,7 +368,7 @@
         else:
             gemm(0, 1, T, Fh, E, h1, E, w1, E, hid, Fh, bias=b1, flags=N.GEMM_RELU, drop_p=drop_p, seed=s_ffn)
         ff = _empty((T, E), x)
-        gemm(0, 1, T, E, Fh, hid, Fh, w2, Fh, ff, E, bias=b2)
+        gemm_w(1, T, E, Fh, hid, Fh, w2, Fh, ff, E, bias=b2)
         y = _empty((T, E), x)
         st2 = _empty((T, 2), x)
         call("rlt_add_layernorm_fwd", ptr(h1), ptr(ff), ptr(n2_w), ptr(n2_b), T, E, eps, drop_p, s_ln2, ptr(y), ptr(st2), stream())
@@ -395,7 +408,7 @@
             gemm(0, 0, T, Fh, E, dr2, E, w2, Fh, dhid, Fh, relu_mask=hid, ldmask=Fh, mask_scale=1.0 / (1.0 - drop_p))
         dw1, db1 = _empty((Fh, E), x), _empty((Fh,), x)
         gemm(1, 0, Fh, E, T, dhid, Fh, h1, E, dw1, E, colsum_a=db1)
-        gemm(0, 0, T, E, Fh, dhid, Fh, w1, E, dz2, E, flags=N.GEMM_ACCUMULATE)
+        gemm_w(0, T, E, Fh, dhid, Fh, w1, E, dz2, E, flags=N.GEMM_ACCUMULATE)
         del dhid
         dz1, dr1, dn1_w, dn1_b = ln_bwd(x, proj, n1_w, st1, dz2, s_ln1)
         dw_o, db_o = _empty((E, E), x), _empty((E,), x)
@@ -414,7 +427,7 @@
         ctx.images = None
         dw_in, db_in = _empty((3 * E, E), x), _empty((3 * E,), x)
         gemm(1, 0, 3 * E, E, T, dqkv, 3 * E, x, E, dw_in, E, colsum_a=db_in)
-        gemm(0, 0, T, E, 3 * E, dqkv, 3 * E, in_w, E, dz1, E, flags=N.GEMM_ACCUMULATE)
+        gemm_w(0, T, E, 3 * E, dqkv, 3 * E, in_w, E, dz1, E, flags=N.GEMM_ACCUMULATE)
         return (dz1, dw_in, db_in, dw_o, db_o, dn1_w, dn1_b, dw1, db1, dw2, db2, dn2_w, dn2_b,
                 None, None, None, None, None, None)
 
```

Result: no change. 24780 lists/s, median of 6 (+0.3%).
